# simonkosina/vbt

Measured on AMD Instinct MI355X. Metric: frames/sec end-to-end (detect+NMS+track), EfficientDet-Lite0 320x320, higher is better.
Workload: dtype int8

## Files before the change

### include/vbt_hip_diag.h

```cpp
#ifndef VBT_HIP_DIAG_H
#define VBT_HIP_DIAG_H

#include "vbt_hip.h"

#ifdef __cplusplus
extern "C" {
#endif

#define VBT_MODEL_NO_FUSION 1
#define VBT_MODEL_NO_MBCONV_FUSION 2
#define VBT_MODEL_NO_SEPCONV_FUSION 4
#define VBT_MODEL_NO_NODE_FUSION 16
#define VBT_MODEL_SINGLE_STREAM 32
#define VBT_MODEL_NO_GRAPH 64
#define VBT_MODEL_NO_HEAD_BATCHING 128
#define VBT_MODEL_NO_STEM_FUSION 256
#define VBT_MODEL_CHUNK48 2048
#define VBT_MODEL_IMAGE_BLOCKS 512
#define VBT_MODEL_TILE128 16384
#define VBT_MODEL_NO_BAND 8192
#define VBT_MODEL_NO_EXPDW 4096
#define VBT_MODEL_NO_PW_MERGE 32768
#define VBT_MODEL_NO_AUTOTUNE 8

int vbt_model_tensor_materialized(const vbt_model* m, int tensor_id);
int vbt_model_num_launches(const vbt_model* m);

int vbt_model_read_tensor(vbt_model* m, int tensor_id, int B, int8_t* host_out);

typedef struct {
  int group, alt, step;
  int chosen;
  int variant;
  int first_op, last_op;
  char family[32];
  int n_variants;
  int variants[48];
} vbt_plan_step_space;
int vbt_model_plan_space(const vbt_model* m, vbt_plan_step_space* out, int cap, int* n);

int vbt_streams_share_queue(void* a, void* b, int us, int* shared);

typedef struct {
  char name[32];
  int launches;
  double algorithmic_bytes;
  double macs;
} vbt_kernel_stat;
int vbt_model_kernel_stats(const vbt_model* m, int B, vbt_kernel_stat* out, int cap, int* n);
typedef struct {
  char family[32];
  int op, first_op, variant;
  double ms, algorithmic_bytes, macs;
} vbt_step_time;
int vbt_model_profile_steps(vbt_model* m, const uint8_t* frames_dev, int B, int reps, void* stream, vbt_step_time* out, int cap, int* n);
int vbt_model_profile_overlap(vbt_model* m, int B, int reps, int nstreams, float* single_ms, float* conc_ms, int cap, int* n);

int vbt_model_profile(vbt_model* m, const uint8_t* frames_dev, int B, int reps, void* stream,
                      double* ms_out, int cap);

int vbt_model_profile_families(vbt_model* m, int B, int reps, void* stream, double* ms_out, int cap);

int vbt_overlay_geometry(vbt_overlay* o, int32_t* out, int cap, int* n);
int vbt_overlay_hud_table(vbt_overlay* o, int32_t* out , int cap, int* P);

int vbt_mjpeg_decode_stage_ms(vbt_mjpeg_decoder* d, float* ms6);
int vbt_mjpeg_decode_entropy_info(vbt_mjpeg_decoder* d, int32_t* info4, void* stream);

#ifdef __cplusplus
}
#endif
#endif
```

### vbt_amd/_lib.py

```python
import ctypes
import os

_HERE = os.path.dirname(os.path.abspath(__file__))
LIB_PATH = os.environ.get("VBT_LIB_PATH") or os.path.join(_HERE, "libvbt_hip.so")
_lib = None

c_void_p, c_int, c_char_p, c_double = ctypes.c_void_p, ctypes.c_int, ctypes.c_char_p, ctypes.c_double


class VbtError(RuntimeError):
    pass


class VbtArgError(VbtError, ValueError):
    """VBT_ERR_ARG: the library refused an argument (also a ValueError, like the host-side checks of the wrappers)."""


class TrackerParams(ctypes.Structure):
    _fields_ = [("max_age", ctypes.c_int32), ("min_hits", ctypes.c_int32), ("delta_t", ctypes.c_int32),
                ("asso", ctypes.c_int32), ("iou_threshold", c_double), ("inertia", c_double), ("det_thresh", c_double)]


class Run(ctypes.Structure):
    _fields_ = [("clip", ctypes.c_int32), ("slot0", ctypes.c_int32), ("slot_stride", ctypes.c_int32), ("n_frames", ctypes.c_int32),
# ... 16 lines not shown
                ("strict_placement", ctypes.c_int32), ("model_flags", ctypes.c_int32), ("detection_threshold", ctypes.c_float),
                ("group", ctypes.c_int32), ("plate_diameter", c_double), ("diff_threshold", c_double), ("min_distance", c_double),
                ("tracker", TrackerParams)]


class PipelineInfo(ctypes.Structure):
    _fields_ = [(k, ctypes.c_int32) for k in ("n_slots", "n_clips", "rows_cap", "device", "depth", "ring", "defer", "tracker_inline", "image_size",
                                               "frame_count", "steps_enqueued", "placement_ok", "queue_groups_seen", "group", "next_slot")] + \
               [("reserved", ctypes.c_int32 * 1), ("det_streams", c_void_p * 8), ("copy_stream", c_void_p), ("tracker_stream", c_void_p),
                ("h2d_bytes", ctypes.c_uint64), ("step_host_ns", ctypes.c_uint64), ("step_calls", ctypes.c_uint64)]


class EvalSummary(ctypes.Structure):
    _fields_ = [(k, ctypes.c_int32) for k in ("n_rows", "n_pos", "n_neg", "n_pr", "n_roc", "flags")] + [("ap", c_double), ("auc", c_double)]


class OverlayParams(ctypes.Structure):
    _fields_ = [("trail", ctypes.c_int32), ("thickness", ctypes.c_int32), ("radius", ctypes.c_int32), ("label_scale", ctypes.c_int32),
                ("rgb", ctypes.c_uint8 * 3), ("label", ctypes.c_uint8), ("box", ctypes.c_uint8), ("reserved", ctypes.c_uint8 * 3)]


class OverlayHudParams(ctypes.Structure):
    _fields_ = [("x", ctypes.c_int32), ("y", ctypes.c_int32), ("scale", ctypes.c_int32), ("full_scale_cm", ctypes.c_int32),
                ("bg", ctypes.c_uint8 * 3), ("reserved", ctypes.c_uint8 * 5)]


class FigureParams(ctypes.Structure):
    _fields_ = [(k, ctypes.c_int32) for k in ("width", "height", "scale", "thickness", "max_figures", "max_rows", "max_phases", "reserved")]


class CurveFigureParams(ctypes.Structure):
    _fields_ = [(k, ctypes.c_int32) for k in ("width", "height", "scale", "thickness", "max_figures", "max_series", "max_points", "max_marks")]


class CurveFigureDesc(ctypes.Structure):
    _fields_ = [(k, ctypes.c_int32) for k in ("n_series", "n_marks", "legend_corner", "minor_x", "minor_y")] + \
               [("reserved", ctypes.c_int32 * 3), ("x_title", ctypes.c_char * 32), ("y_title", ctypes.c_char * 32)]


class CurveSeries(ctypes.Structure):
    _fields_ = [("n_points", ctypes.c_int32), ("colour", ctypes.c_int32), ("text", ctypes.c_char * 64)]


class CurveMark(ctypes.Structure):
    _fields_ = [("series", ctypes.c_int32), ("point", ctypes.c_int32), ("text", ctypes.c_char * 16)]


class KernelStat(ctypes.Structure):
    _fields_ = [("name", ctypes.c_char * 32), ("launches", c_int), ("algorithmic_bytes", c_double), ("macs", c_double)]


class StepTime(ctypes.Structure):
    _fields_ = [("family", ctypes.c_char * 32), ("op", c_int), ("first_op", c_int), ("variant", c_int), ("ms", c_double),
                ("algorithmic_bytes", c_double), ("macs", c_double)]


class PlanStepSpace(ctypes.Structure):
    _fields_ = [("group", c_int), ("alt", c_int), ("step", c_int), ("chosen", c_int), ("variant", c_int), ("first_op", c_int),
                ("last_op", c_int), ("family", ctypes.c_char * 32),
                ("n_variants", c_int), ("variants", c_int * 48)]


_SIGS = {
    "vbt_last_error": (c_char_p, []),
    "vbt_device_count": (c_int, []),
    "vbt_model_create": (c_int, [c_char_p, c_int, c_int, ctypes.POINTER(c_void_p)]),
    "vbt_model_create_ex": (c_int, [c_char_p, c_int, c_int, c_int, ctypes.POINTER(c_void_p)]),
    "vbt_model_destroy": (None, [c_void_p]),
    "vbt_model_tensor_materialized": (c_int, [c_void_p, c_int]),
    "vbt_model_num_launches": (c_int, [c_void_p]),
    "vbt_model_input_shape": (c_int, [c_void_p, ctypes.POINTER(c_int)]),
    "vbt_model_num_tensors": (c_int, [c_void_p]),
    "vbt_model_num_ops": (c_int, [c_void_p]),
    "vbt_model_tensor_shape": (c_int, [c_void_p, c_int, ctypes.POINTER(c_int)]),
    "vbt_detect": (c_int, [c_void_p, c_void_p, c_int, c_int, c_void_p, c_void_p, c_void_p, c_void_p, c_void_p, c_int]),
    "vbt_detect_async": (c_int, [c_void_p, c_void_p, c_int, c_void_p, c_void_p, c_void_p, c_void_p, c_void_p]),
    "vbt_detect_range_async": (c_int, [c_void_p, c_void_p, c_int, c_int, c_int, c_int, c_void_p, c_void_p, c_void_p, c_void_p, c_void_p]),
    "vbt_model_entry_steps": (c_int, [c_void_p]),
    "vbt_stream_create": (c_int, [c_int, c_void_p]),
    "vbt_stream_destroy": (c_int, [c_void_p]),
    "vbt_streams_share_queue": (c_int, [c_void_p, c_void_p, c_int, c_void_p]),
    "vbt_model_read_tensor": (c_int, [c_void_p, c_int, c_int, c_void_p]),
    "vbt_model_plan_space": (c_int, [c_void_p, c_void_p, c_int, ctypes.POINTER(c_int)]),
    "vbt_resize_frames": (c_int, [c_void_p, c_int, c_int, c_int, c_int, c_void_p, c_int, c_int, c_int, c_int, c_int, c_void_p]),
    "vbt_resize_frames_yuv": (c_int, [c_void_p, c_int, c_int, c_int, c_int, c_int, c_void_p, c_int, c_int, c_int, c_int, c_void_p]),
    "vbt_model_kernel_stats": (c_int, [c_void_p, c_int, ctypes.POINTER(KernelStat), c_int, ctypes.POINTER(c_int)]),
    "vbt_model_profile": (c_int, [c_void_p, c_void_p, c_int, c_int, c_void_p, ctypes.POINTER(c_double), c_int]),
    "vbt_model_profile_families": (c_int, [c_void_p, c_int, c_int, c_void_p, ctypes.POINTER(c_double), c_int]),
    "vbt_model_profile_steps": (c_int, [c_void_p, c_void_p, c_int, c_int, c_void_p, ctypes.POINTER(StepTime), c_int, ctypes.POINTER(c_int)]),
    "vbt_model_profile_overlap": (c_int, [c_void_p, c_int, c_int, c_int, c_void_p, c_void_p, c_int, c_void_p]),
    "vbt_tracker_create": (c_int, [c_int, c_int, ctypes.POINTER(TrackerParams), c_int, ctypes.POINTER(c_void_p)]),
    "vbt_tracker_destroy": (None, [c_void_p]),
    "vbt_tracker_reset": (c_int, [c_void_p]),
    "vbt_tracker_reset_clips": (c_int, [c_void_p, c_void_p, c_int, c_void_p]),
    "vbt_tracker_update": (c_int, [c_void_p, c_void_p, c_void_p, c_void_p, c_int]),
    "vbt_tracker_update_from_detections": (c_int, [c_void_p, c_void_p, c_void_p, c_void_p, c_void_p, ctypes.c_float, c_void_p]),
    "vbt_tracker_last_output": (c_int, [c_void_p, c_int, c_void_p, c_void_p, c_int, ctypes.POINTER(c_int)]),
    "vbt_tracker_get_trackers": (c_int, [c_void_p, c_int, c_void_p, c_void_p, c_int, ctypes.POINTER(c_int)]),
    "vbt_tracker_status": (c_int, [c_void_p, c_int] + [ctypes.POINTER(ctypes.c_int32)] * 5),
    "vbt_tracker_rows": (c_int, [c_void_p, c_int, c_void_p, c_void_p, c_int, ctypes.POINTER(c_int)]),
    "vbt_tracker_finish": (c_int, [c_void_p, c_double, c_double, c_double, c_void_p]),
    "vbt_tracker_phases": (c_int, [c_void_p, c_int, ctypes.POINTER(ctypes.c_int32), c_void_p, c_int, ctypes.POINTER(c_int)]),
    "vbt_tracker_update_from_slots": (c_int, [c_void_p, c_void_p, c_void_p, c_void_p, c_void_p, c_void_p, c_int, ctypes.c_float, c_void_p]),
    "vbt_tracker_update_from_detections_seq": (c_int, [c_void_p, c_void_p, c_void_p, c_void_p, c_int, c_void_p, c_int, ctypes.c_float, c_void_p]),
    "vbt_gather_frames": (c_int, [c_void_p, c_void_p, c_int, ctypes.c_size_t, c_void_p]),
    "vbt_tracker_summary": (c_int, [c_void_p, c_void_p, c_void_p, c_void_p, c_void_p, c_void_p, c_int]),
    "vbt_tracker_rows_all": (c_int, [c_void_p, c_void_p, c_void_p, c_int, c_void_p]),
    "vbt_tracker_live_enable": (c_int, [c_void_p, c_int, c_int, c_double, c_double, c_double]),
    "vbt_tracker_live_poll": (c_int, [c_void_p, c_int, c_void_p, c_void_p, c_int, c_void_p]),
    "vbt_tracker_live_tracks": (c_int, [c_void_p, c_int, c_int, c_void_p, c_void_p, c_void_p, c_void_p, c_void_p, c_int, c_int, ctypes.POINTER(c_int)]),
    "vbt_pipeline_default_params": (None, [ctypes.POINTER(PipelineParams)]),
    "vbt_pipeline_create": (c_int, [c_char_p, ctypes.POINTER(PipelineParams), c_void_p, ctypes.POINTER(c_void_p)]),
    "vbt_pipeline_destroy": (None, [c_void_p]),
    "vbt_pipeline_step": (c_int, [c_void_p, c_void_p, c_int, c_int, c_int, c_int, c_void_p, c_void_p, c_void_p, c_int, c_void_p]),
    "vbt_pipeline_step_runs": (c_int, [c_void_p, c_void_p, c_void_p, c_int, c_void_p, c_int, c_int, c_int, c_int, c_int, c_void_p, c_void_p, c_void_p,
                                       c_void_p, c_void_p]),
    "vbt_pipeline_set_pixel_format": (c_int, [c_void_p, c_int]),
    "vbt_pipeline_skip_frames": (c_int, [c_void_p, c_int]),
    "vbt_pipeline_set_frame_count": (c_int, [c_void_p, c_int]),
    "vbt_pipeline_reset": (c_int, [c_void_p]),
    "vbt_pipeline_join_detectors": (c_int, [c_void_p, c_void_p]),
    "vbt_pipeline_close": (c_int, [c_void_p, c_void_p, c_void_p, c_void_p, c_void_p, c_void_p, c_int]),
    "vbt_pipeline_finish": (c_int, [c_void_p]),
    "vbt_pipeline_close_clips_enable": (c_int, [c_void_p]),
    "vbt_pipeline_close_clips": (c_int, [c_void_p, c_void_p, c_int, c_void_p]),
    "vbt_pipeline_closed_clip": (c_int, [c_void_p, c_int, c_int, ctypes.POINTER(c_int), ctypes.POINTER(ClosedClip), c_void_p, c_int, c_void_p, c_int]),
    "vbt_pipeline_drain": (c_int, [c_void_p]),
    "vbt_pipeline_rows_all": (c_int, [c_void_p, c_void_p, c_void_p, c_int]),
    "vbt_pipeline_rows": (c_int, [c_void_p, c_int, c_void_p, c_void_p, c_int, ctypes.POINTER(c_int)]),
    "vbt_pipeline_detections": (c_int, [c_void_p, c_void_p, c_void_p, c_void_p, c_void_p, c_int, ctypes.POINTER(c_int)]),
    "vbt_pipeline_tracker_only_steps": (c_int, [c_void_p, c_int, c_int]),
    "vbt_pipeline_live_enable": (c_int, [c_void_p, c_int, c_int]),
    "vbt_pipeline_live_poll": (c_int, [c_void_p, c_int, c_void_p, c_void_p, c_int]),
    "vbt_pipeline_get_info": (c_int, [c_void_p, ctypes.POINTER(PipelineInfo)]),
    "vbt_pipeline_model": (c_void_p, [c_void_p, c_int]),
    "vbt_pipeline_tracker": (c_void_p, [c_void_p]),
    "vbt_track_clip": (c_int, [c_void_p, c_void_p, c_int, c_int, c_int, c_int, c_int, c_int, c_void_p, c_void_p, c_int, ctypes.POINTER(c_int)]),
    "vbt_host_alloc": (c_int, [ctypes.c_size_t, ctypes.POINTER(c_void_p)]),
    "vbt_host_free": (c_int, [c_void_p]),
    "vbt_device_alloc": (c_int, [c_int, ctypes.c_size_t, ctypes.POINTER(c_void_p)]),
    "vbt_device_free": (c_int, [c_void_p]),
    "vbt_memcpy": (c_int, [c_void_p, c_void_p, ctypes.c_size_t, c_int]),
    "vbt_stream_synchronize": (c_int, [c_void_p]),
    "vbt_device_synchronize": (c_int, [c_int]),
    "vbt_analyze": (c_int, [c_void_p, c_int, c_int, c_int, c_double, c_double, c_double, c_void_p, c_int, ctypes.POINTER(c_int), c_int]),
    "vbt_window_means": (c_int, [c_void_p, c_int, c_int, c_void_p, c_void_p, c_int]),
    "vbt_eval_create": (c_int, [c_int, c_int, c_int, ctypes.POINTER(c_void_p)]),
    "vbt_eval_destroy": (None, [c_void_p]),
    "vbt_eval_reset": (c_int, [c_void_p]),
    "vbt_eval_add_detections": (c_int, [c_void_p, c_void_p, c_void_p, c_void_p, c_int, c_void_p, c_void_p, c_void_p, c_void_p]),
    "vbt_eval_table": (c_int, [c_void_p, ctypes.POINTER(c_int), c_void_p, c_void_p, c_void_p, c_void_p, c_void_p, c_int]),
    "vbt_eval_curves": (c_int, [c_void_p, c_double, ctypes.POINTER(EvalSummary), c_void_p, c_void_p, c_void_p, c_int, c_void_p, c_void_p, c_void_p, c_int]),
    "vbt_eval_curves_from_table": (c_int, [c_void_p, c_void_p, c_int, c_double, c_int, ctypes.POINTER(EvalSummary), c_void_p, c_void_p, c_void_p, c_int,
                                           c_void_p, c_void_p, c_void_p, c_int]),
    "vbt_overlay_default_params": (None, [ctypes.POINTER(OverlayParams)]),
    "vbt_overlay_create": (c_int, [c_int, c_int, c_int, c_int, ctypes.POINTER(OverlayParams), ctypes.POINTER(c_void_p)]),
    "vbt_overlay_destroy": (None, [c_void_p]),
    "vbt_overlay_set_rows": (c_int, [c_void_p, c_void_p, c_int, c_double, c_void_p]),
    "vbt_overlay_draw": (c_int, [c_void_p, c_void_p, c_int, c_int, c_int, c_void_p]),
    "vbt_overlay_geometry": (c_int, [c_void_p, c_void_p, c_int, ctypes.POINTER(c_int)]),
    "vbt_overlay_hud_default_params": (None, [ctypes.POINTER(OverlayHudParams)]),
    "vbt_overlay_set_hud": (c_int, [c_void_p, ctypes.POINTER(OverlayHudParams), c_void_p, c_int, c_double, c_void_p]),
    "vbt_overlay_hud_table": (c_int, [c_void_p, c_void_p, c_int, ctypes.POINTER(c_int)]),
    "vbt_overlay_hud_follow": (c_int, [c_void_p, ctypes.POINTER(OverlayHudParams), c_void_p, c_int, c_double]),
    "vbt_overlay_hud_follow_update": (c_int, [c_void_p, c_int, c_void_p]),
    "vbt_overlay_hud_follow_status": (c_int, [c_void_p, ctypes.POINTER(ctypes.c_int64), ctypes.POINTER(ctypes.c_int32), ctypes.POINTER(ctypes.c_int32), c_void_p]),
# ... 74 lines not shown
```

### vbt_amd/csrc/detector.hip

```cpp
#include <algorithm>
#include <cmath>

#include "detector_model.h"
#include "op_kernels.h"

namespace vbt {

static_assert(PWM_MAX == PW_MERGE_MAX, "the planner merges as many pointwise convs as one pw_multi_kernel launch takes");


PwLaunch resolve_pw(const vbt_model* m, const Step& s, int variant, int B) {
  PwLaunch L;
  const TensorRec& to = m->tensors[m->ops[s.res_op >= 0 ? s.p_op : s.op].output];
  const long M = (long)B * to.h * to.w;
  if (s.KS64 <= 4) {
    L.form = PW_A;
    L.ms = variant >= 0 ? (variant & 1) + 1 : (M >= 32768 ? 2 : 1);
    const long waves = (M + 16 * L.ms - 1) / (16 * L.ms);
    const unsigned gx = (unsigned)((waves + 3) / 4);
    int ysplit = 1;
    while (gx * ysplit < 1024 && ysplit < s.NB) ysplit++;
    L.nb_per_y = (s.NB + ysplit - 1) / ysplit;
    L.grid = dim3(gx, (s.NB + L.nb_per_y - 1) / L.nb_per_y);
    return L;
  }
  static const int pw_force = getenv("VBT_PW_VARIANT") ? atoi(getenv("VBT_PW_VARIANT")) : -100;
  const bool f_fits = s.NB >= 2 && s.NB <= PW_F_MAX_NB;
  if (pw_force != -100 && (f_fits || (pw_force != 7 && pw_force != 8))) variant = pw_force;
  if (variant == 7 || variant == 8) {
    L.form = PW_F;
    L.ms = variant - 6;
    L.lds = s.NB * 8192;
    L.grid = dim3((unsigned)((M + 64 * L.ms - 1) / (64 * L.ms)), 1);
    if (s.NB < 2) L.refuse(VBT_ERR_ARG, "pw_conv: one output block - nothing for the all-blocks form to share");
    else if (s.NB > PW_F_MAX_NB) L.refuse(VBT_ERR_ARG, "pw_conv: %d output blocks exceed the %d whose accumulators the all-blocks form holds", s.NB, PW_F_MAX_NB);
  } else if (variant >= 3 && variant <= 6) {
    L.form = variant <= 4 ? PW_D : PW_E;
    L.ms = 2 - (variant & 1);
    L.lds = L.form == PW_E ? s.KS64 * 4096 : 0;
    L.grid = dim3((unsigned)((M + 64 * L.ms - 1) / (64 * L.ms)), (unsigned)s.NB);
    if (L.lds > 160 * 1024) L.refuse(VBT_ERR_ARG, "pw_conv: a weight panel of %d bytes does not fit the LDS", L.lds);
  } else if (variant == 2) {
    L.form = PW_C;
    L.ms = ((M + 31) / 32) * s.NB >= 512 ? 2 : 1;
    L.grid = dim3((unsigned)((M + 16 * L.ms - 1) / (16 * L.ms)), (unsigned)s.NB);
  } else {
    const unsigned gx = (unsigned)(((M + 15) / 16 + 3) / 4);
    L.nbt = std::min(s.NB, 4);
    if (gx < 512 && L.nbt > 2) L.nbt = 2;
    if (gx < 128) L.nbt = 1;
    L.grid = dim3(gx, (s.NB + L.nbt - 1) / L.nbt);
  }
  return L;
}
static int launch_pw_step(const vbt_model* m, const Step& s, int B, hipStream_t st, const int8_t* x, const int8_t* res, int8_t* out) {
  const PwLaunch L = resolve_pw(m, s, s.variant, B);
  if (L.rc) return L.report();
  const OpRec& pop = m->ops[s.res_op >= 0 ? s.p_op : s.op];
  const TensorRec& tpo = m->tensors[pop.output];
  const Epi e{s.bias, s.mult, tpo.zero_point, pop.act_min, pop.act_max, make_rq(tpo.zero_point, pop.act_min, pop.act_max)};
  const ResArgs ra{res, s.addq};
  const long M = (long)B * tpo.h * tpo.w;
  const int K = m->tensors[pop.inputs[0]].c, N = tpo.c;
#define PW(KERNEL, LDS) KERNEL<<<L.grid, 256, LDS, st>>>(x, s.wp64, e, ra, out, M, K, s.KS64, N, s.NB)
#define PW_A(KS) (L.ms == 2 ? pw_a_kernel<KS, 2><<<L.grid, 256, 0, st>>>(x, s.wp64, e, ra, out, M, K, N, s.NB, L.nb_per_y) \
                            : pw_a_kernel<KS, 1><<<L.grid, 256, 0, st>>>(x, s.wp64, e, ra, out, M, K, N, s.NB, L.nb_per_y))
  switch (L.form) {
    case PW_A: if (s.KS64 == 1) PW_A(1); else if (s.KS64 == 2) PW_A(2); else if (s.KS64 == 3) PW_A(3); else PW_A(4); break;
    case PW_D: if (L.ms == 2) PW(pw_d_kernel<2>, 0); else PW(pw_d_kernel<1>, 0); break;
    case PW_C: if (L.ms == 2) PW((pw_c_kernel<1, 2>), 0); else PW((pw_c_kernel<1, 1>), 0); break;
    case PW_E:
      if (L.ms == 2) { if (L.lds > 64 * 1024) VBT_LDS_OPT_IN(pw_e_kernel<2, 4>); PW((pw_e_kernel<2, 4>), L.lds); }
      else { if (L.lds > 64 * 1024) VBT_LDS_OPT_IN(pw_e_kernel<1, 4>); PW((pw_e_kernel<1, 4>), L.lds); }
      break;
    case PW_F:
#define PW_F_NB(NBF) (L.ms == 2 ? PW((pw_f_kernel<NBF, 2, 4>), 0) : PW((pw_f_kernel<NBF, 1, 4>), 0))
      if (s.NB == 2) PW_F_NB(2); else if (s.NB == 3) PW_F_NB(3); else if (s.NB == 4) PW_F_NB(4); else if (s.NB == 5) PW_F_NB(5); else PW_F_NB(6);
#undef PW_F_NB
      break;
    case PW_B:
      if (L.nbt == 1) PW(pw_b_kernel<1>, 0); else if (L.nbt == 2) PW(pw_b_kernel<2>, 0); else if (L.nbt == 3) PW(pw_b_kernel<3>, 0); else PW(pw_b_kernel<4>, 0);
      break;
  }
#undef PW
#undef PW_A
  return VBT_OK;
}

DwLaunch resolve_dw(const vbt_model* m, const Step& s, int variant, int B) {
  DwLaunch L;
  const OpRec& op = m->ops[s.op];
  const TensorRec& to = m->tensors[op.output];
  if (variant == 100 || variant == 101) {
    L.form = DW_TILE; L.mdw = variant == 101;
    choose_tile(to.h, to.w, op.k, op.stride, false, &L.TX, &L.TY);
    L.tiles_x = (to.w + L.TX - 1) / L.TX;
    L.tiles_y = (to.h + L.TY - 1) / L.TY;
    const int TXp = (L.TX + 3) & ~3;
    L.lds = ((TXp - 1) * op.stride + op.k) * ((L.TY - 1) * op.stride + op.k) * 80;
    L.grid = dim3((unsigned)((long)B * L.tiles_x * L.tiles_y), (unsigned)((to.c + 63) / 64));
  } else if (variant == 0) {
    L.form = DW_ROW;
    L.total = (long)B * to.h * ((to.w + 3) / 4) * (to.c / 4);
    L.grid = dim3((unsigned)((L.total + 255) / 256));
  } else {
    const long per_seg = (long)B * ((to.w + 3) / 4) * (to.c / 4);
    L.rows = std::min(variant > 0 ? variant : (int)std::min<long>(std::max<long>(to.h * per_seg / 400000, 1), 16), to.h);
    L.nseg = (to.h + L.rows - 1) / L.rows;
    L.total = per_seg * L.nseg;
    L.grid = dim3((unsigned)((L.total + 255) / 256));
  }
  return L;
}
static int launch_dw_step(const vbt_model* m, const Step& s, int B, hipStream_t st, const int8_t* x, int8_t* out, const Epi& e) {
  const DwLaunch L = resolve_dw(m, s, s.variant, B);
  if (L.rc) return L.report();
  const OpRec& op = m->ops[s.op];
  const TensorRec& ti = m->tensors[op.inputs[0]];
  const TensorRec& to = m->tensors[op.output];
  if (L.form == DW_TILE) {
    DwTileArgs a;
    a.x = x; a.out = out; a.wf = s.wf; a.bias = s.bias; a.mult = s.mult; a.wdm = s.wdm; a.bdm = s.bdm; a.mdm = s.mdm;
    a.H = ti.h; a.W = ti.w; a.C = to.c; a.OH = to.h; a.OW = to.w; a.pad_t = op.pad_t; a.pad_l = op.pad_l;
    a.TX = L.TX; a.TY = L.TY; a.tiles_x = L.tiles_x; a.tiles_y = L.tiles_y; a.zx = ti.zero_point; a.rq = e.rq;
    return launch_dw_tile(a, op.k, op.stride, L.mdw, L.grid, L.lds, st);
  }
  const unsigned pb = (unsigned)((128 + ti.zero_point) & 255);
  const unsigned pad4 = pb | (pb << 8) | (pb << 16) | (pb << 24);
#define DW_LAUNCH(KERNEL, ...)                                                                    \
  do {                                                                                            \
    if (op.k == 3 && op.stride == 1) KERNEL<3, 1><<<L.grid, 256, 0, st>>>(__VA_ARGS__);           \
    else if (op.k == 3 && op.stride == 2) KERNEL<3, 2><<<L.grid, 256, 0, st>>>(__VA_ARGS__);      \
    else if (op.k == 5 && op.stride == 1) KERNEL<5, 1><<<L.grid, 256, 0, st>>>(__VA_ARGS__);      \
    else KERNEL<5, 2><<<L.grid, 256, 0, st>>>(__VA_ARGS__);                                       \
  } while (0)
  if (L.form == DW_ROW) DW_LAUNCH(dw_kernel, x, s.wf, e, out, L.total, ti.h, ti.w, to.c, to.h, to.w, op.pad_t, op.pad_l, pad4);
  else DW_LAUNCH(dw_col_kernel, x, s.wf, e, out, L.total, ti.h, ti.w, to.c, to.h, to.w, op.pad_t, op.pad_l, pad4, L.rows, L.nseg);
#undef DW_LAUNCH
  return VBT_OK;
}

FusedPlan resolve_fused(const vbt_model* m, const Step& s, int variant, int B) {
  const FusedArgs& a = s.fa;
  const OpRec& dop = m->ops[s.d_op];
  const int k = dop.k, stride = dop.stride;
  const bool ex = s.family == F_MBCONV, ks12 = a.KSe == 1 || a.KSe == 2;
  int var = variant;
  if (var < 0) {
    var = ((m->flags & VBT_MODEL_IMAGE_BLOCKS) && !resolve_fused(m, s, 5, B).rc) ? 5 : ((m->flags & VBT_MODEL_CHUNK48) ? 9 : 1);
    const FusedPlan p17 = (m->flags & VBT_MODEL_TILE128) ? resolve_fused(m, s, 17, B) : FusedPlan{};
    if (!p17.rc && p17.L.ppw2) var |= 16;
  }
  const bool mdw = var & 1, half = var & 2;
  const bool nt3 = (var & 8) && mdw && a.nch3 > 0 && s.nbp <= 2 && a.KSe >= 1 && a.KSe <= 4;
  FusedPlan p;
  if ((var & 32) && (var & 4)) { p.refuse(VBT_ERR_ARG, "fused_mbconv: variant %d: the Toeplitz depthwise does not apply to this step", var); return p; }
  if (var & 4) {
    const int HW = a.H * a.W, OHW = a.OH * a.OW;
    if (!ex || HW > 400 || OHW > 400 || !s.ib.data) { p.refuse(VBT_ERR_ARG, "fused_mbconv: whole-image variant not applicable"); return p; }
    p.image = true;
    p.PH = std::max((a.OH - 1) * stride + k, a.pad_t + a.H);
    p.PW = std::max((a.OW - 1) * stride + k, a.pad_l + a.W);
    p.NB = (a.Cout + 63) / 64;
    const int NPGo = (OHW + 15) / 16;
    const int units = (NPGo * p.NB + IB_WAVES - 1) / IB_WAVES;
    p.maxu = units <= 2 ? 2 : units <= 3 ? 3 : 4;
    p.L.k = k; p.L.stride = stride; p.L.lds_bytes = ((HW * a.T0S + 15) & ~15) + p.PH * p.PW * FB_EST + NPGo * 16 * FB_DST + s.ib.bytes;
    if (units > 4 || p.L.lds_bytes > 160 * 1024 || s.ib.bytes > 16 * IB_NPF * IB_THREADS) p.refuse(VBT_ERR_ARG, "fused_mbconv: whole-image variant not applicable");
    return p;
  }
  p.TX = a.TX;
  p.TY = half && a.TY >= 2 ? (a.TY + 1) / 2 : a.TY;
  const bool ppw2 = (var & 16) && ex && mdw && ks12 && s.nbp <= 2 && !half;
  if (ppw2) { p.TX = 16; p.TY = 8; }
  const bool dw64 = ppw2 || (ex && mdw && a.wd64 && p.TX == 8 && p.TY == 8 && ks12 && s.nbp <= 2);
  const int est = !ex ? 0 : !nt3 ? FB_EST : dw64 ? 48 : 72;
  const bool tpz = var & 32;
  const bool tpz_ok = tpz && dw64 && a.wtz && fused_tpz_built(k, stride, s.nbp, a.KSe, ppw2) && (var & ~(1 | 8 | 16 | 32)) == 0 && nt3 == bool(var & 8) && ppw2 == bool(var & 16);
  const TpzGeom tg = tpz_ok ? tpz_geom(k, stride, ppw2 ? 2 : 1, nt3 ? 3 : 4) : TpzGeom{};
  const int e_bytes = tpz_ok ? tg.e_bytes + 8 * tg.DSK : -1;
  p.tiles_x = (a.OW + p.TX - 1) / p.TX;
  p.tiles_y = (a.OH + p.TY - 1) / p.TY;
  p.L = FusedLaunch{k, stride, s.nbp, ex, mdw, nt3, ppw2, dw64, fused_tile_lds(a, k, stride, p.TX, p.TY, est, ppw2 ? 2 : 1, s.nbp, e_bytes),
                    (unsigned)((long)B * p.tiles_x * p.tiles_y), tpz_ok};
  if (ppw2 && (a.OW < 16 || a.OH < 8 || !a.wd64)) p.refuse(VBT_ERR_ARG, "fused_mbconv: the 128-pixel variant needs maps of at least 16 x 8");
  else if (ppw2 && p.L.lds_bytes > 64 * 1024) p.refuse(VBT_ERR_ARG, "fused_mbconv: 128-pixel tile needs %d bytes of LDS", p.L.lds_bytes);
  else if (tpz && !tpz_ok) p.refuse(VBT_ERR_ARG, "fused_mbconv: variant %d: the Toeplitz depthwise does not apply to this step", var);
  else if (tpz && p.L.lds_bytes > 64 * 1024) p.refuse(VBT_ERR_ARG, "fused_mbconv: the Toeplitz depthwise tile needs %d bytes of LDS", p.L.lds_bytes);
  return p;
}
static int launch_fused_step(const vbt_model* m, const Step& s, FusedArgs a, int B, hipStream_t st) {
  const FusedPlan p = resolve_fused(m, s, s.variant, B);
  if (p.rc) return p.report();
  if (p.image) return launch_mbconv_image(a, s.ib, p.L.k, p.L.stride, p.maxu, p.PW, p.PH, p.NB, p.L.lds_bytes, B, st);
  a.TX = p.TX; a.TY = p.TY; a.tiles_x = p.tiles_x; a.tiles_y = p.tiles_y;
  return launch_fused_block(a, p.L, st);
}

ExpDwLaunch resolve_expdw(const vbt_model*, const Step& s, int variant, int B) {
  static const int xd_force = getenv("VBT_XD_VARIANT") ? atoi(getenv("VBT_XD_VARIANT")) : -100;
  if (xd_force != -100 && (xd_force < 100 || (s.xd2_ok && (xd_force < 200 ? s.xd2_gpw > 0 : s.xd2_gpw16 > 0)))) variant = std::min(xd_force, xd_force / 100 * 100 + s.xd.nchunks);
  ExpDwLaunch L;
  if (s.xd2_ok && (variant >= 100 || variant < 0)) {
    if (variant >= 200 && s.xd2_gpw16 == 0) { L.refuse(VBT_ERR_ARG, "expand + depthwise: plan asks for the 16-wave form on a step that does not support it"); return L; }
    if (variant >= 100 && variant < 200 && s.xd2_gpw == 0) { L.refuse(VBT_ERR_ARG, "expand + depthwise: plan asks for the 8-wave form on a step that does not support it"); return L; }
    const ExpDw2Args& a = s.xd2;
    L.second = true;
    L.nw = (variant >= 200 || (variant < 0 && s.xd2_gpw16 > 0)) ? 16 : 8;
    L.gpw = L.nw == 16 ? s.xd2_gpw16 : s.xd2_gpw;
    L.cpw = std::min(variant >= 100 ? variant % 100 : std::max(1, (a.nchunks * a.nbands * B + 1023) / 1024), a.nchunks);
    L.grid = (unsigned)(B * ((a.nchunks + L.cpw - 1) / L.cpw) * a.nbands);
    L.lds = s.xd2_lds;
    return L;
  }
  if (variant >= 100) { L.refuse(VBT_ERR_ARG, "expand + depthwise: plan asks for the second kernel form on a step that does not support it"); return L; }
  const ExpDwArgs& a = s.xd;
  L.cpw = variant > 0 ? variant : std::max(1, (a.nchunks * a.nbands * B + 511) / 512);
  L.grid = (unsigned)(B * ((a.nchunks + L.cpw - 1) / L.cpw) * a.nbands);
  L.lds = s.lds_bytes;
  return L;
}
static int launch_expdw_step(const vbt_model* m, const Step& s, int B, hipStream_t st, const int8_t* x, int8_t* out) {
  const ExpDwLaunch L = resolve_expdw(m, s, s.variant, B);
  if (L.rc) return L.report();
  const OpRec& dop = m->ops[s.d_op];
  if (L.second) {
    ExpDw2Args a = s.xd2;
    a.x = x; a.out = out; a.cpw = L.cpw;
    return launch_expdw2(a, dop.k, dop.stride, (a.Cin + 63) / 64, L.nw, L.gpw, L.grid, L.lds, st);
  }
  ExpDwArgs a = s.xd;
  a.x = x; a.out = out; a.cpw = L.cpw;
  return launch_expdw(a, dop.k, dop.stride, (a.Cin + 63) / 64, L.grid, L.lds, st);
}

static bool band_chainable(const Step& s) {
  if (s.members.empty()) return s.bd_args.wpc != nullptr;
  for (const Step& ms : s.members)
    if (!ms.bd_args.wpc) return false;
  return true;
}
BandLaunch resolve_band(const vbt_model* m, const Step& s, int variant, int) {
  BandLaunch L;
  const bool can = band_chainable(s);
  if (variant < -1 || variant > 1) { L.refuse(VBT_ERR_ARG, "fused_sepconv_band: no kernel form %d", variant); return L; }
  if (variant == 1 && !can) { L.refuse(VBT_ERR_ARG, "fused_sepconv_band: plan asks for the chained form on a step that does not support it"); return L; }
  static const int bd_force = getenv("VBT_BAND_VARIANT") ? atoi(getenv("VBT_BAND_VARIANT")) : -100;
  if (bd_force == 0 || (bd_force == 1 && can)) variant = bd_force;
  L.chained = variant == 1 || (variant < 0 && can && m->max_batch > 8);
  if (s.members.empty()) L.lds = band_lds(s.bd_args, L.chained);
  for (const Step& ms : s.members) L.lds = std::max(L.lds, band_lds(ms.bd_args, L.chained));
  if (L.lds > 160 * 1024) L.refuse(VBT_ERR_ARG, "fused_sepconv_band: a band of %d bytes does not fit the LDS", L.lds);
  return L;
}

StemLaunch resolve_stemblk(const vbt_model*, const Step&, int variant, int) {
  StemLaunch L;
  if (variant < -1 || variant > 1) { L.refuse(VBT_ERR_ARG, "fused_stem_block: no kernel form %d", variant); return L; }
  L.direct = variant == 1;
  return L;
}

int launch_step(vbt_model* m, const Step& s, int B, hipStream_t st, const uint8_t* frames, float* boxes, float* scores, float* classes,
                int* counts, int boff) {
  if (m->pool_dirty) { const int rc = flush_uploads(m); if (rc) return rc; }
  const OpRec& op = m->ops[s.op];
  const TensorRec& to = m->tensors[op.output];
// ... 356 lines not shown
```

### vbt_amd/csrc/detector_model.h

```cpp
#pragma once
#include <cstdarg>
#include <map>
#include <tuple>
#include <vector>

#include "dev_mem.h"
#include "hip_handles.h"
#include "launchers.h"
#include "plan_geom.h"

namespace vbt {

enum Family { F_STEM = 0, F_PW, F_DW, F_ADD, F_MAXPOOL, F_RESIZE, F_POST, F_MBCONV, F_SEPCONV, F_NODE, F_MULTI, F_STEMBLK, F_EXPDW, F_BAND, F_COUNT };
inline const char* const kFamilyName[F_COUNT] = {"stem_conv_mfma_i8", "pw_conv_mfma_i8", "dw_conv_f32acc", "add_requant",
                                                 "maxpool3x3s2", "resize_nn", "decode_nms", "fused_mbconv", "fused_sepconv", "fused_bifpn_node", "fused_heads_multi",
                                                 "fused_stem_block", "fused_expand_dw", "fused_sepconv_band"};

constexpr int PW_MERGE_MAX = 8;

struct Cost {
  double alg_bytes_per_frame = 0, weight_bytes = 0, macs_per_frame = 0;
  Cost& operator+=(const Cost& o) { alg_bytes_per_frame += o.alg_bytes_per_frame; weight_bytes += o.weight_bytes; macs_per_frame += o.macs_per_frame; return *this; }
};

struct Step {
  int op;
  int family;
  long* wp = nullptr;
  v4i* wp64 = nullptr;
  int KS64 = 0;
  int res_op = -1;
  long* wdm = nullptr;
  int* bdm = nullptr;
  float* mdm = nullptr;
  float* wf = nullptr;
  int* bias = nullptr;
  float* mult = nullptr;
  int KS = 0, NB = 0;
  AddQ addq = {0, 0, 0, 0, 0, 0, 0};
  Cost cost;
  int e_op = -1, d_op = -1, p_op = -1, a_op = -1;
  int sum_op = -1;
  int src_tensor[3] = {-1, -1, -1};
  FusedArgs fa;
  int nbp = 0, lds_bytes = 0;
  int variant = -1;
  double tuned_ms = 0;
  std::vector<Step> members;
  FusedArgs* d_multi = nullptr;
  StemBlockArgs sb;
  BandArgs bd_args;
  BandArgs* d_band = nullptr;
  int band_tiles = 0;
  ExpDwArgs xd;
  ExpDw2Args xd2;
  bool xd2_ok = false;
  int xd2_lds = 0, xd2_gpw = 0, xd2_gpw16 = 0;
  ImageBundle ib = {nullptr, 0, 0, 0, 0, 0, 0, 0};
};

struct Alt {
  std::vector<Step> steps;
  std::vector<int> hidden;
  double ms = 0;
};
struct Group {
  std::vector<Alt> alts;
  int chosen = 0;
};

}

struct vbt_model {
  vbt_model() = default;
  ~vbt_model() {
    for (int k = 0; k < 4; k++) { sub_streams[k].reset(); ev_join[k].reset(); }
    ev_fork.reset();
    clear_graphs();
    cap_stream.reset();
  }
  vbt::Header hdr;
  std::vector<vbt::TensorRec> tensors;
  std::vector<vbt::OpRec> ops;
  std::vector<uint8_t> blob;
  int device = 0, max_batch = 0;
  std::vector<int8_t*> tptr;
  std::vector<size_t> telems;
  int8_t* arena = nullptr;
  uint8_t* frames_stage = nullptr;
  vbt::DevBuf<unsigned char> out_block;
  float* out_boxes = nullptr;
  float* out_scores = nullptr;
  float* out_classes = nullptr;
  int* out_counts = nullptr;
  vbt::PinnedBuf<unsigned char> out_host;
  size_t out_bytes = 0;
  float* d_anchors = nullptr;
  unsigned char* d_luts = nullptr;
  std::vector<float> post_tables_host;
  std::vector<vbt::Step> steps;
  std::vector<vbt::Group> groups;
  std::vector<vbt::Step> op_steps;
  std::vector<char> materialized;
  int flags = 0;
  int n_sub = 1;
  vbt::Stream sub_streams[4];
  vbt::Event ev_fork, ev_join[4];
  struct GraphKey {
    const void* frames; void* boxes; void* scores; void* classes; void* counts; int B;
    bool operator<(const GraphKey& o) const {
      return std::tie(frames, boxes, scores, classes, counts, B) < std::tie(o.frames, o.boxes, o.scores, o.classes, o.counts, o.B);
    }
  };
  std::map<GraphKey, hipGraphExec_t> graphs;
  void clear_graphs() {
    for (auto& kv : graphs) (void)hipGraphExecDestroy(kv.second);
    graphs.clear();
  }
  vbt::Stream cap_stream;
  int graph_max_batch = 0;
  bool ran_eager = false;
  std::vector<vbt::DevBuf<char>> owned;
  struct PoolChunk { vbt::DevBuf<char> dev; std::vector<char> host; size_t used, flushed; };
  std::vector<PoolChunk> pool;
  bool pool_dirty = false;
  int last_B = 0;
};

namespace vbt {

int upload_bytes(vbt_model* m, const void* src, size_t bytes, void** dev);
template <typename T>
int upload(vbt_model* m, const std::vector<T>& h, T** d) { return upload_bytes(m, h.data(), h.size() * sizeof(T), (void**)d); }
int flush_uploads(vbt_model* m);

int build_plan(vbt_model* m);
void finalize_plan(vbt_model* m);

struct Verdict {
  int rc = VBT_OK; char why[160] = "";
  void refuse(int code, const char* fmt, ...) { va_list ap; va_start(ap, fmt); vsnprintf(why, sizeof(why), fmt, ap); va_end(ap); rc = code; }
  int report() const { set_error("%s", why); return rc; }
};
enum PwForm { PW_A, PW_B, PW_C, PW_D, PW_E, PW_F };
constexpr int PW_F_MAX_NB = 6;
struct PwLaunch : Verdict { PwForm form = PW_B; int ms = 1, nbt = 1, nb_per_y = 0, lds = 0; dim3 grid; };
enum DwForm { DW_ROW, DW_COL, DW_TILE };
struct DwLaunch : Verdict {
  DwForm form = DW_COL; bool mdw = false; int TX = 0, TY = 0, tiles_x = 0, tiles_y = 0, lds = 0, rows = 0, nseg = 0; long total = 0; dim3 grid;
};
struct FusedPlan : Verdict {
  bool image = false; int PW = 0, PH = 0, NB = 0, maxu = 0;
  int TX = 0, TY = 0, tiles_x = 0, tiles_y = 0; FusedLaunch L{};
};
struct ExpDwLaunch : Verdict {
  bool second = false; int cpw = 1, nw = 0, gpw = 0, lds = 0; unsigned grid = 0;
};
struct BandLaunch : Verdict { bool chained = false; int lds = 0; };
struct StemLaunch : Verdict { bool direct = false; };
PwLaunch resolve_pw(const vbt_model* m, const Step& s, int variant, int B);
DwLaunch resolve_dw(const vbt_model* m, const Step& s, int variant, int B);
FusedPlan resolve_fused(const vbt_model* m, const Step& s, int variant, int B);
ExpDwLaunch resolve_expdw(const vbt_model* m, const Step& s, int variant, int B);
BandLaunch resolve_band(const vbt_model* m, const Step& s, int variant, int B);
StemLaunch resolve_stemblk(const vbt_model* m, const Step& s, int variant, int B);

int launch_step(vbt_model* m, const Step& s, int B, hipStream_t st, const uint8_t* frames, float* boxes, float* scores, float* classes,
                int* counts, int boff = 0);
inline int launch_step_staged(vbt_model* m, const Step& s, int B, hipStream_t st) {
  return launch_step(m, s, B, st, m->frames_stage, m->out_boxes, m->out_scores, m->out_classes, m->out_counts);
}
int enqueue_forward(vbt_model* m, const uint8_t* frames_dev, int B, hipStream_t st, float* boxes, float* scores, float* classes, int* counts,
                    const Event* evs);

}
```

### vbt_amd/csrc/detector_plan.hip

```cpp
#include <algorithm>
#include <chrono>
#include <cmath>
#include <functional>
#include <string>

#include "detector_model.h"

namespace vbt {

static bool fence_on() {
  static int v = -1;
  if (v < 0) { const char* e = getenv("VBT_DEBUG_FENCE"); v = (e && e[0] == '1') ? 1 : 0; }
  return v == 1;
}
static hipError_t fenced_malloc(vbt_model* m, void** out, size_t bytes) {
  const size_t G = 2u << 20;
  const size_t total = fence_on() ? (bytes + G - 1) / G * G : bytes;
  DevBuf<char> base;
  const hipError_t e = base.alloc(total);
  if (e != hipSuccess) return e;
  *out = base.get() + ((total - bytes) & ~(size_t)255);
  m->owned.push_back(std::move(base));
  return hipSuccess;
}
// ... 17 lines not shown
  return VBT_OK;
}
int flush_uploads(vbt_model* m) {
  if (!m->pool_dirty) return VBT_OK;
  for (auto& c : m->pool)
    if (c.used > c.flushed) {
      VBT_HIP_CHECK(hipMemcpy(c.dev.get() + c.flushed, c.host.data() + c.flushed, c.used - c.flushed, hipMemcpyHostToDevice));
      c.flushed = c.used;
    }
  m->pool_dirty = false;
  return VBT_OK;
}

int upload_bytes(vbt_model* m, const void* src, size_t n, void** d) {
  size_t bytes = std::max<size_t>(n, 16);
  if (fence_on()) {
    VBT_HIP_CHECK(fenced_malloc(m, d, bytes + 64));
    if (n) VBT_HIP_CHECK(hipMemcpy(*d, src, n, hipMemcpyHostToDevice));
    return VBT_OK;
  }
  char* host = nullptr;
  int rc = pool_alloc(m, bytes + 64, d, &host);
  if (rc) return rc;
  if (n) memcpy(host, src, n);
  return VBT_OK;
}

static double time_step(vbt_model* m, const Step& s, int B, int reps) {
  static int nconc = -1;
  static hipStream_t cs[4] = {nullptr, nullptr, nullptr, nullptr};
  if (nconc < 0) {
    const char* e = getenv("VBT_AUTOTUNE_CONCURRENCY");
    nconc = e ? std::max(1, std::min(4, atoi(e))) : 1;
    if (nconc > 1)
      for (int i = 0; i < nconc; i++) (void)hipStreamCreateWithFlags(&cs[i], hipStreamNonBlocking);
  }
  Event e0, e1;
  if (e0.create(hipEventDefault) != hipSuccess || e1.create(hipEventDefault) != hipSuccess) return 1e30;
  float ms = 1e30f;
  int rc = VBT_OK;
  if (nconc <= 1) {
    rc = launch_step_staged(m, s, B, nullptr);
    (void)hipEventRecord(e0.get(), nullptr);
    for (int r = 0; r < reps && !rc; r++)
      rc = launch_step_staged(m, s, B, nullptr);
    (void)hipEventRecord(e1.get(), nullptr);
    if (hipEventSynchronize(e1.get()) != hipSuccess || hipEventElapsedTime(&ms, e0.get(), e1.get()) != hipSuccess) ms = 1e30f;
    ms /= reps;
  } else {
    (void)hipDeviceSynchronize();
    for (int i = 0; i < nconc && !rc; i++)
      rc = launch_step_staged(m, s, B, cs[i]);
    (void)hipDeviceSynchronize();
    auto t0 = std::chrono::steady_clock::now();
    for (int r = 0; r < reps; r++)
      for (int i = 0; i < nconc && !rc; i++)
        rc = launch_step_staged(m, s, B, cs[i]);
    (void)hipDeviceSynchronize();
    ms = (float)(std::chrono::duration<double, std::milli>(std::chrono::steady_clock::now() - t0).count() / (reps * nconc));
  }
  return rc ? 1e30 : ms;
}

static bool is_fused_tile(int family) { return family == F_MBCONV || family == F_SEPCONV || family == F_NODE; }
static bool variant_ok(const vbt_model* m, const Step& st, int v) {
  if (st.family == F_PW) return !st.members.empty() || !resolve_pw(m, st, v, m->max_batch).rc;
  if (is_fused_tile(st.family)) return !resolve_fused(m, st, v, m->max_batch).rc;
  if (st.family == F_BAND) return !resolve_band(m, st, v, m->max_batch).rc;
  if (st.family == F_STEMBLK) return !resolve_stemblk(m, st, v, m->max_batch).rc;
  return st.family != F_EXPDW || !resolve_expdw(m, st, v, m->max_batch).rc;
}

static std::vector<int> candidate_variants(const vbt_model* m, const Step& st) {
  std::vector<int> cand{-1};
  const OpRec& op = m->ops[st.op];
  if (st.family == F_DW) {
    cand = {0};
    for (int r : {1, 2, 4, 8, 16})
      if (r <= m->tensors[op.output].h) cand.push_back(r);
    if (m->tensors[op.output].c % 8 == 0) { cand.push_back(100); cand.push_back(101); }
  } else if (st.family == F_PW && st.KS64 <= 4) {
    cand = {0, 1};
  } else if (st.family == F_PW) {
    cand = {-1, 2, 3, 4, 5, 6, 7, 8};
  } else if (is_fused_tile(st.family)) {
    cand = {0, 1, 3, 5};
    if (st.family == F_MBCONV && st.fa.nch3 > 0 && st.nbp <= 2 && st.fa.KSe >= 1 && st.fa.KSe <= 4) { cand.push_back(9); cand.push_back(11); }
    if (st.family == F_MBCONV && st.nbp <= 2 && (st.fa.KSe == 1 || st.fa.KSe == 2)) {
      cand.push_back(17);
      if (st.fa.nch3 > 0) cand.push_back(25);
    }
    if (st.family == F_MBCONV && st.fa.wtz) cand.insert(cand.end(), {33, 41, 49, 57});
  } else if (st.family == F_MULTI) {
    cand = {0, 1};
  } else if (st.family == F_EXPDW) {
    cand.clear();
    for (int cpw : {1, 2, 3, 4, 6})
      if (cpw <= st.xd.nchunks) cand.push_back(cpw);
    if (st.xd2_ok)
      for (int cpw : {1, 2, 3, 4, 6})
        if (cpw <= st.xd.nchunks) {
          if (st.xd2_gpw > 0) cand.push_back(100 + cpw);
          if (st.xd2_gpw16 > 0) cand.push_back(200 + cpw);
        }
  } else if (st.family == F_BAND) {
    cand = {-1, 0, 1};
  } else if (st.family == F_STEMBLK) {
    cand = {-1, 0, 1};
  }
  cand.erase(std::remove_if(cand.begin(), cand.end(), [&](int v) { return !variant_ok(m, st, v); }), cand.end());
  return cand;
}

static void autotune(vbt_model* m) {
  const int B = (m->max_batch + m->n_sub - 1) / m->n_sub, reps = 4;
  for (Group& g : m->groups) {
    bool single = g.alts.size() == 1 && g.alts[0].steps.size() == 1;
    if (single) {
      int f = g.alts[0].steps[0].family;
      if (f != F_DW && f != F_PW) continue;
    }
    for (Alt& a : g.alts) {
      a.ms = 0;
      for (Step& st : a.steps) {
        const std::vector<int> cand = candidate_variants(m, st);
        double best = 1e30;
        int bestv = -1;
        for (int v : cand) {
          Step t = st;
          t.variant = v;
          double ms = time_step(m, t, B, reps);
          if (getenv("VBT_AUTOTUNE_VERBOSE") && cand.size() > 1 && atoi(getenv("VBT_AUTOTUNE_VERBOSE")) > 1)
            fprintf(stderr, "[autotune]   op %d %s v%d %.1fus\n", st.op, kFamilyName[st.family], v, ms * 1e3);
          if (ms < best) { best = ms; bestv = v; }
        }
        st.variant = bestv;
        st.tuned_ms = best;
        a.ms += best;
      }
    }
    int bi = 0;
    for (size_t i = 1; i < g.alts.size(); i++)
      if (g.alts[i].ms < g.alts[bi].ms) bi = (int)i;
    g.chosen = bi;
    if (getenv("VBT_AUTOTUNE_VERBOSE")) {
      const Step& f = g.alts[0].steps[0];
      const TensorRec& to = m->tensors[m->ops[g.alts[0].steps.back().op].output];
      fprintf(stderr, "[autotune] op %3d.. out %3dx%3dx%4d :", f.op, to.h, to.w, to.c);
      for (size_t i = 0; i < g.alts.size(); i++) {
        fprintf(stderr, " alt%zu%s %.1fus(", i, (int)i == bi ? "*" : "", g.alts[i].ms * 1e3);
        for (const Step& st : g.alts[i].steps) fprintf(stderr, "%s:v%d=%.1f ", kFamilyName[st.family], st.variant, st.tuned_ms * 1e3);
        fprintf(stderr, ")");
      }
      fprintf(stderr, "\n");
    }
  }
  (void)hipDeviceSynchronize();
}

static PlanShape plan_shape(const vbt_model* m) {
  PlanShape shape;
  for (const Group& g : m->groups) {
    std::vector<std::vector<PlanStepShape>> alts;
    for (const Alt& a : g.alts) {
      std::vector<PlanStepShape> steps;
      for (const Step& st : a.steps) {
        PlanStepShape ps;
// ... 13 lines not shown
  return shape;
}
static bool load_plan(vbt_model* m, const char* path) {
  const PlanShape shape = plan_shape(m);
  std::vector<PlanChoice> sel;
  std::string note;
  if (!parse_plan_file(path, shape, &sel, &note)) {
    if (note != "no such file") fprintf(stderr, "[vbt] plan %s: %s - plan refused, re-tuning\n", path, note.c_str());
    return false;
  }
  for (size_t gi = 0; gi < m->groups.size(); gi++) {
    m->groups[gi].chosen = sel[gi].chosen;
    Alt& a = m->groups[gi].alts[(size_t)sel[gi].chosen];
    for (size_t i = 0; i < a.steps.size(); i++) a.steps[i].variant = sel[gi].variants[i];
  }
  return true;
}
static void save_plan(const vbt_model* m, const char* path) {
  FILE* f = fopen(path, "w");
  if (!f) return;
  fprintf(f, "VBTPLAN2 %d\n", (int)m->groups.size());
  for (const Group& g : m->groups) {
    const Alt& a = g.alts[g.chosen];
    fprintf(f, "%d %d", g.chosen, (int)a.steps.size());
    for (const Step& st : a.steps) fprintf(f, " %s:%d", kFamilyName[st.family], st.variant);
    fprintf(f, "\n");
  }
  fclose(f);
}

}

using namespace vbt;

extern "C" {

int vbt_model_create(const char* path, int device, int max_batch, vbt_model** out) {
  const char* nf = getenv("VBT_FUSION_FLAGS");
  return vbt_model_create_ex(path, device, max_batch, nf ? atoi(nf) : VBT_MODEL_DEFAULT_FLAGS, out);
}

int vbt_model_tensor_materialized(const vbt_model* m, int id) {
  if (!m || id < 0 || id >= (int)m->tensors.size()) { set_error("bad tensor id"); return VBT_ERR_ARG; }
  return m->materialized[id] ? 1 : 0;
}

int vbt_model_num_launches(const vbt_model* m) { return m ? (int)m->steps.size() : VBT_ERR_ARG; }

int vbt_model_plan_space(const vbt_model* m, vbt_plan_step_space* out, int cap, int* n) {
  if (!m || !n || cap < 0 || (cap > 0 && !out)) { set_error("vbt_model_plan_space: bad argument"); return VBT_ERR_ARG; }
  const PlanShape shape = plan_shape(m);
  int total = 0;
  for (const auto& alts : shape.groups)
    for (const auto& steps : alts) total += (int)steps.size();
  *n = total;
  if (total > cap) { set_error("plan space: %d steps, buffer holds %d", total, cap); return VBT_ERR_CAPACITY; }
  int i = 0;
  for (size_t gi = 0; gi < shape.groups.size(); gi++)
    for (size_t ai = 0; ai < shape.groups[gi].size(); ai++)
      for (size_t si = 0; si < shape.groups[gi][ai].size(); si++, i++) {
        const PlanStepShape& ps = shape.groups[gi][ai][si];
        vbt_plan_step_space& o = out[i];
        memset(&o, 0, sizeof(o));
        if (ps.variants.size() > sizeof(o.variants) / sizeof(o.variants[0])) {
          set_error("plan space: group %zu alternative %zu step %zu has %zu variants", gi, ai, si, ps.variants.size());
          return VBT_ERR_CAPACITY;
        }
        o.group = (int)gi; o.alt = (int)ai; o.step = (int)si;
        o.chosen = m->groups[gi].chosen == (int)ai;
        const Step& st = m->groups[gi].alts[ai].steps[si];
        o.variant = st.variant;
        o.first_op = (int)m->ops.size(); o.last_op = -1;
        std::function<void(const Step&)> span = [&](const Step& s) {
          for (int op : {s.op, s.e_op, s.d_op, s.p_op, s.a_op, s.sum_op})
            if (op >= 0) { o.first_op = std::min(o.first_op, op); o.last_op = std::max(o.last_op, op); }
          for (const Step& mb : s.members) span(mb);
        };
        span(st);
        snprintf(o.family, sizeof(o.family), "%s", ps.family.c_str());
        o.n_variants = (int)ps.variants.size();
        std::copy(ps.variants.begin(), ps.variants.end(), o.variants);
      }
  return VBT_OK;
}

int vbt_model_create_ex(const char* path, int device, int max_batch, int flags, vbt_model** out) {
  if (!path || !out || max_batch < 1) { set_error("vbt_model_create: bad argument"); return VBT_ERR_ARG; }
  *out = nullptr;
  vbt_model* m = new vbt_model();
  {
    ContainerData cd;
    std::string why;
    if (!read_container(path, &cd, &why)) { delete m; set_error("%s", why.c_str()); return VBT_ERR_IO; }
    m->hdr = cd.hdr;
    m->tensors.swap(cd.tensors);
    m->ops.swap(cd.ops);
    m->blob.swap(cd.blob);
  }
  m->device = device;
  m->max_batch = max_batch;
  m->flags = flags;
  if (int drc = use_device("vbt_model_create", device, false)) { delete m; return drc; }
  int rc = VBT_OK;
  auto fail = [&](int code) { vbt_model_destroy(m); return code; };
  if (hipSetDevice(device) != hipSuccess) { set_error("hipSetDevice(%d) failed", device); return fail(VBT_ERR_HIP); }
  size_t total = 0;
  m->telems.resize(m->tensors.size());
  std::vector<size_t> off(m->tensors.size());
  for (size_t i = 0; i < m->tensors.size(); i++) {
    const TensorRec& t = m->tensors[i];
    m->telems[i] = (size_t)t.h * t.w * t.c;
    off[i] = total;
    size_t bytes = (int)i == m->hdr.input_tensor ? 0 : m->telems[i] * max_batch;
    total += (bytes + 255) / 256 * 256 + 256;
  }
  if (fenced_malloc(m, (void**)&m->arena, total + 4096) != hipSuccess) { set_error("hipMalloc(%zu) for activations failed", total); return fail(VBT_ERR_HIP); }
  (void)hipMemset(m->arena, 0, total + 4096);
  m->tptr.resize(m->tensors.size());
  for (size_t i = 0; i < m->tensors.size(); i++) m->tptr[i] = m->arena + off[i];
  size_t fbytes = (size_t)max_batch * m->hdr.image_size * m->hdr.image_size * 3;
  const int md = m->hdr.max_detections;
  m->out_bytes = (size_t)max_batch * (md * 24 + 4);
  if (fenced_malloc(m, (void**)&m->frames_stage, fbytes + 64) != hipSuccess || m->out_block.alloc(m->out_bytes) != hipSuccess ||
      m->out_host.alloc(m->out_bytes) != hipSuccess) {
    set_error("hipMalloc for staging buffers failed");
    return fail(VBT_ERR_HIP);
  }
  m->out_boxes = (float*)m->out_block.get();
  m->out_scores = m->out_boxes + (size_t)max_batch * md * 4;
  m->out_classes = m->out_scores + (size_t)max_batch * md;
  m->out_counts = (int*)(m->out_classes + (size_t)max_batch * md);
  if ((rc = build_plan(m)) != VBT_OK) return fail(rc);
  for (const OpRec& op : m->ops)
    if (op.type == OP_POSTPROCESS) {
      std::vector<float> an((const float*)(m->blob.data() + op.aux_off), (const float*)(m->blob.data() + op.aux_off) + (size_t)m->hdr.num_anchors * 4);
      if ((size_t)op.aux2_off + VBT_POST_TABLE_BYTES > m->blob.size()) { set_error("post-process tables truncated"); return fail(VBT_ERR_IO); }
      std::vector<unsigned char> lut(m->blob.data() + op.aux2_off, m->blob.data() + op.aux2_off + VBT_POST_TABLE_BYTES);
      const float* sv = (const float*)(lut.data() + 6144);
      if (sv[0] != sv[1] || sv[2] != sv[3]) { set_error("post-process: y_scale != x_scale or h_scale != w_scale"); return fail(VBT_ERR_ARG); }
      {
        const int nl = op.n_inputs / 2;
        const TensorRec& tc = m->tensors[op.inputs[0]];
        const TensorRec& tb = m->tensors[op.inputs[nl]];
        for (int l = 1; l < nl; l++) {
          const TensorRec &c2 = m->tensors[op.inputs[l]], &b2 = m->tensors[op.inputs[nl + l]];
          if (c2.scale != tc.scale || c2.zero_point != tc.zero_point || b2.scale != tb.scale || b2.zero_point != tb.zero_point) {
            set_error("post-process: head outputs of level %d are quantised differently from level 0", l);
            return fail(VBT_ERR_ARG);
          }
        }
        const float* st_score = (const float*)lut.data();
        const float* st_box = st_score + 256;
        const double* st_dq = (const double*)(lut.data() + 2048);
        const double* st_ex = st_dq + 256;
        for (int q = -128; q < 128; q++) {
          const float x = tc.scale * (float)(q - tc.zero_point);
          float y = 256.0f / (1.0f + expf(-x));
          y = y < 0.0f ? 0.0f : (y > 255.0f ? 255.0f : y);
          const float want_score = (1.0f / 256.0f) * (float)lrintf(y);
          const float want_box = tb.scale * (float)(q - tb.zero_point);
          const double want_dq = (double)want_box / (double)sv[0];
          const double want_ex = exp((double)want_box / (double)sv[2]);
          if (st_score[q + 128] != want_score || st_box[q + 128] != want_box || st_dq[q + 128] != want_dq || st_ex[q + 128] != want_ex) {
            set_error("post-process: stored table entry %d differs from the one derived from the tensor scales", q);
            return fail(VBT_ERR_ARG);
          }
// ... 73 lines not shown
```

### vbt_amd/csrc/fused_block.h

```cpp
#pragma once
#include "tpz_geom.h"

struct FusedArgs {
  const int8_t* x;
  int8_t* out;
  int H, W, Cin, OH, OW, Cout;
  int pad_t, pad_l;
  int TX, TY, tiles_x, tiles_y;
  int T0S;
  int nchunks;
  int zx;
  const long* we;
  const int* be;
  const float* me;
  int KSe, ze, loe, hie;
  Rq rqe;
  const long* we3;
  const long* wdm3;
  const v4i* wp3;
  int nch3, KSp3;
  const float* wd;
  const int* bd;
  const float* md;
  int zd, lod, hid;
  Rq rqd;
  const long* wdm;
  const int* bdm;
  const v4i* wd64;
  const long* wd64c;
  const unsigned* wtz;
  const v4i* wp;
  const int* bp;
  const float* mp;
  int KSp, zo, lop, hip;
  Rq rqp;
  int has_res;
  AddQ resq;
  int n_src;
  const int8_t* src[3];
  int sh[3], sw[3], smode[3], spt[3], spl[3];
  int chain;
  AddQ sumq, preq;
};

__device__ __forceinline__ unsigned node_sum4(const unsigned u[3], const FusedArgs& a) {
  if (a.chain == 0) return addq4(u[0], u[1], a.sumq);
  const unsigned p = addq4(u[0], u[1], a.preq);
  return a.chain == 1 ? addq4(p, u[2], a.sumq) : addq4(u[2], p, a.sumq);
}

typedef unsigned short v2u16 __attribute__((ext_vector_type(2)));
__device__ __forceinline__ unsigned pk_max_u16(unsigned a, unsigned b) {
  v2u16 x, y;
  __builtin_memcpy(&x, &a, 4);
  __builtin_memcpy(&y, &b, 4);
  v2u16 r = __builtin_elementwise_max(x, y);
  unsigned o;
  __builtin_memcpy(&o, &r, 4);
  return o;
}

constexpr int FB_EST = 80;
constexpr int FB_DST = 80;

template <int KK, int S, int NBP, bool EXPAND, bool MDW, int KSE = 0, int NT = 4, int PPW = 1, bool DW64 = false, bool TPZ = false>
__device__ __forceinline__ void fused_block_body(const FusedArgs& a, int tile, unsigned char* fb_smem) {
  static_assert(PPW == 1 || MDW, "128-pixel tiles exist for the matrix-pipe depthwise only");
  static_assert(!DW64 || (EXPAND && MDW && (KK == 3 || KK == 5)), "DW64: fused expand blocks, 3x3 / 5x5");
  static_assert(!TPZ || (DW64 && (S == 1 || S == 2) && (NT == 3 || NT == 4) && NBP <= 2 && (KSE == 1 || KSE == 2)), "TPZ: a form of DW64");
  constexpr TpzGeom TG = TPZ ? tpz_geom(KK, S, PPW, NT) : TpzGeom{};
  constexpr int KT2 = (S * (S - 1) + KK + 1) / 2;
  const int tid = threadIdx.x, wave = tid >> 6, lane = tid & 63, r = lane & 15, g = lane >> 4;
  const int trow = fdiv_small(tile, frcp(a.tiles_x));
  const int tx = tile - trow * a.tiles_x;
  const int bimg = fdiv_small(trow, frcp(a.tiles_y));
  const int ty = trow - bimg * a.tiles_y;
  const long b = bimg;
  const int oy0 = ty * a.TY, ox0 = tx * a.TX;
  const int TXp = (a.TX + 3) & ~3;
  const int HWx = (TXp - 1) * S + KK, HWy = (a.TY - 1) * S + KK, NPh = HWx * HWy;
  const int iy0 = oy0 * S - a.pad_t, ix0 = ox0 * S - a.pad_l;
  const float rcp_hwx = frcp(HWx), rcp_txp = frcp(TXp);
  unsigned char* T0 = fb_smem;
  unsigned char* E = T0 + ((NPh * a.T0S + 15) & ~15);
  constexpr int EST = (EXPAND && NT == 3) ? (DW64 ? 48 : 72) : FB_EST;
  unsigned char* D = E + (EXPAND ? (TPZ ? TG.e_bytes : ((NPh * EST + 15) & ~15)) : 0);
  bool stage_p = false;
  if constexpr (!EXPAND && NBP <= 2) stage_p = a.nchunks == 1;
  unsigned char* WPS = D + 64 * PPW * FB_DST;
  unsigned char* BPS = WPS + NBP * 4096;

  bool summed = false;
  if constexpr (!EXPAND) summed = a.n_src > 0;
  if (summed) {
    const int nd = a.Cin >> 2;
    const unsigned zb4 = (unsigned)(a.zx & 255) * 0x01010101u;
    const int pstep = fdiv_small(256, frcp(nd));
    int p = fdiv_small(tid, frcp(nd));
    const int cd = tid - p * nd;
    const bool up2[3] = {a.H == 2 * a.sh[0] && a.W == 2 * a.sw[0], a.H == 2 * a.sh[1] && a.W == 2 * a.sw[1], a.H == 2 * a.sh[2] && a.W == 2 * a.sw[2]};
    for (; tid < pstep * nd && p < NPh; p += pstep) {
      const int hy = fdiv_small(p, rcp_hwx), hx = p - hy * HWx;
      const int iy = iy0 + hy, ix = ix0 + hx;
      unsigned v = zb4;
      if (iy >= 0 && iy < a.H && ix >= 0 && ix < a.W) {
        unsigned us[3] = {0u, 0u, 0u};
#pragma unroll
        for (int j = 0; j < 3; j++) {
          if (j < a.n_src) {
            const int8_t* sb = a.src[j] + b * (long)a.sh[j] * a.sw[j] * a.Cin + 4 * cd;
            unsigned u;
            if (a.smode[j] == 0) {
              u = *(const unsigned*)(sb + ((long)iy * a.sw[j] + ix) * a.Cin);
            } else if (a.smode[j] == 1) {
              int yy, xx;
              if (up2[j]) { yy = iy >> 1; xx = ix >> 1; }
              else { yy = (iy * a.sh[j]) / a.H; xx = (ix * a.sw[j]) / a.W; }
              u = *(const unsigned*)(sb + ((long)yy * a.sw[j] + xx) * a.Cin);
            } else {
              unsigned tv[9];
#pragma unroll
              for (int ky = 0; ky < 3; ky++) {
                const int yy = iy * 2 + ky - a.spt[j];
                const int yc = min(max(yy, 0), a.sh[j] - 1);
#pragma unroll
                for (int kx = 0; kx < 3; kx++) {
                  const int xx = ix * 2 + kx - a.spl[j];
                  const int xc = min(max(xx, 0), a.sw[j] - 1);
                  const unsigned t = *(const unsigned*)(sb + ((long)yc * a.sw[j] + xc) * a.Cin);
                  tv[ky * 3 + kx] = (yy == yc && xx == xc) ? (t ^ 0x80808080u) : 0u;
                }
              }
              unsigned lo = 0u, hi = 0u;
#pragma unroll
              for (int q = 0; q < 9; q++) {
                const unsigned l = tv[q] & 0x00FF00FFu, h = (tv[q] >> 8) & 0x00FF00FFu;
                lo = pk_max_u16(lo, l);
                hi = pk_max_u16(hi, h);
              }
              u = (lo | (hi << 8)) ^ 0x80808080u;
            }
            us[j] = u;
          }
        }
        v = node_sum4(us, a);
      }
      *(unsigned*)(T0 + p * a.T0S + 4 * cd) = v;
    }
  } else {
    if (!EXPAND && (a.Cin & 15) == 0) {
// ... 260 lines not shown
      if (PREF_DW || (!EXPAND && c == 0)) {
#pragma unroll
        for (int mi = 0; mi < KT; mi++) wreg[mi] = wpre[mi];
        bqm = bpre;
        mum = mpre;
      } else if (cg_active) {
#pragma unroll
        for (int mi = 0; mi < KT; mi++) wreg[mi] = wm[mi * 64];
        bqm = *(const int4*)(a.bdm + c * CH + 16 * wave + 4 * g);
        mum = *(const float4*)(a.md + c * CH + 16 * wave + 4 * g);
      }
      const unsigned char* lane_base = Ein + 16 * wave + 8 * (g & 1);
      const int hi_half = g >> 1;
#pragma unroll
      for (int pg = 0; pg < 4 * PPW; pg += 2) {
        if (!cg_active) break;
        v4i dqa = v4i_from(bqm), dqb = v4i_from(bqm);
        const unsigned char* pba = lane_base + hbase[pg] * est;
        const unsigned char* pbb = lane_base + hbase[pg + 1] * est;
#pragma unroll
        for (int mi = 0; mi < KT; mi++) {
          const int ta = 2 * mi, tb = (2 * mi + 1 < KK * KK) ? 2 * mi + 1 : 2 * mi;
          const int offa = ((ta / KK) * HWx + (ta % KK)) * est, offb = ((tb / KK) * HWx + (tb % KK)) * est;
          const int off = hi_half ? offb : offa;
          long bva = *(const long*)(pba + off);
          long bvb = *(const long*)(pbb + off);
          dqa = __builtin_amdgcn_mfma_i32_16x16x32_i8(wreg[mi], bva, dqa, 0, 0, 0);
          dqb = __builtin_amdgcn_mfma_i32_16x16x32_i8(wreg[mi], bvb, dqb, 0, 0, 0);
        }
        *(unsigned*)(D + (pg * 16 + r) * FB_DST + 16 * wave + 4 * g) = rq_pack_b(dqa, mum, a.rqd);
        *(unsigned*)(D + ((pg + 1) * 16 + r) * FB_DST + 16 * wave + 4 * g) = rq_pack_b(dqb, mum, a.rqd);
      }
    } else if (dw_active) {
      const unsigned char* Ein = EXPAND ? E + 4 * cq : T0 + 64 * c + 4 * cq;
      const int est = EXPAND ? EST : a.T0S;
      constexpr int IW = 3 * S + KK;
      const int Cp = a.nchunks * 64;
      const float* wd = a.wd + c * 64 + 4 * cq;
      float dacc[4][4];
#pragma unroll
      for (int o = 0; o < 4; o++)
#pragma unroll
        for (int j = 0; j < 4; j++) dacc[o][j] = 0.0f;
#pragma unroll
      for (int ky = 0; ky < KK; ky++) {
        float4 wr[KK];
#pragma unroll
        for (int kx = 0; kx < KK; kx++) wr[kx] = *(const float4*)(wd + (long)(ky * KK + kx) * Cp);
        const unsigned char* rowp = Ein + ((sy * S + ky) * HWx + sx * S) * est;
#pragma unroll
        for (int j = 0; j < IW; j++) {
          unsigned u = *(const unsigned*)(rowp + j * est) ^ 0x80808080u;
          float f0 = (float)(u & 255u), f1 = (float)((u >> 8) & 255u), f2 = (float)((u >> 16) & 255u), f3 = (float)(u >> 24);
#pragma unroll
          for (int kx = 0; kx < KK; kx++) {
            if ((j - kx) >= 0 && (j - kx) % S == 0 && (j - kx) / S < 4) {
              const int o = (j - kx) / S;
              dacc[o][0] = __builtin_fmaf(f0, wr[kx].x, dacc[o][0]);
              dacc[o][1] = __builtin_fmaf(f1, wr[kx].y, dacc[o][1]);
              dacc[o][2] = __builtin_fmaf(f2, wr[kx].z, dacc[o][2]);
              dacc[o][3] = __builtin_fmaf(f3, wr[kx].w, dacc[o][3]);
            }
          }
        }
      }
      const int4 bq = *(const int4*)(a.bd + c * 64 + 4 * cq);
      const float4 mu = *(const float4*)(a.md + c * 64 + 4 * cq);
#pragma unroll
      for (int o = 0; o < 4; o++) {
        v4i ai = {(int)dacc[o][0], (int)dacc[o][1], (int)dacc[o][2], (int)dacc[o][3]};
        unsigned dd = rq_pack_i(ai, bq, mu, a.rqd);
        *(unsigned*)(D + (sy * TXp + sx + o) * FB_DST + 4 * cq) = dd;
      }
    }
    __syncthreads();
    {
      v4i bv[PPW];
#pragma unroll
      for (int pp = 0; pp < PPW; pp++) {
        const int slot = (wave * PPW + pp) * 16 + r;
        bv[pp] = *(const v4i*)(D + (TPZ ? tpz_d_slot(TG, PPW, FB_DST, slot) : slot * FB_DST) + 16 * g);
      }
#pragma unroll
      for (int nb = 0; nb < NBP; nb++) {
        const v4i* w = stage_p ? (const v4i*)WPS + (nb * 4) * 64 + lane
                               : (NT == 3 ? a.wp3 + ((long)(nb * a.KSp3 + c) * 4) * 64 : a.wp + ((long)(nb * a.KSp + c) * 4) * 64) + lane;
#pragma unroll
        for (int t = 0; t < 4; t++) {
          const v4i wv = w[t * 64];
#pragma unroll
          for (int pp = 0; pp < PPW; pp++) acc[pp][nb][t] = __builtin_amdgcn_mfma_i32_16x16x64_i8(wv, bv[pp], acc[pp][nb][t], 0, 0, 0);
        }
      }
    }
    if (!EXPAND && c + 1 < nch) __syncthreads();
  }

#pragma unroll
  for (int pp = 0; pp < PPW; pp++) {
  const int slot = (wave * PPW + pp) * 16 + r;
  const int py = fdiv_small(slot, rcp_txp), px = slot - py * TXp;
  const int oy = oy0 + py, ox = ox0 + px;
  if (py < a.TY && px < a.TX && oy < a.OH && ox < a.OW) {
    const unsigned char* skip = T0 + ((py + a.pad_t) * HWx + (px + a.pad_l)) * a.T0S;
    int8_t* orow = a.out + ((b * a.OH + oy) * (long)a.OW + ox) * a.Cout;
#pragma unroll
    for (int nb = 0; nb < NBP; nb++) {
      const int c0 = nb * 64 + 16 * g;
      if (c0 >= a.Cout) continue;
      unsigned d[4];
#pragma unroll
      for (int t = 0; t < 4; t++) {
        int4 bb;
        float4 mu;
        if (stage_p) {
          bb = *(const int4*)(BPS + 4 * (c0 + 4 * t));
          mu = *(const float4*)(BPS + NBP * 256 + 4 * (c0 + 4 * t));
        } else {
          bb = *(const int4*)(a.bp + c0 + 4 * t);
          mu = *(const float4*)(a.mp + c0 + 4 * t);
        }
        unsigned dq = rq_pack_i(acc[pp][nb][t], bb, mu, a.rqp);
        if (a.has_res) {
          const unsigned xs = *(const unsigned*)(skip + min(c0 + 4 * t, a.Cin - 4));
          dq = addq4(dq, xs, a.resq);
        }
        d[t] = dq;
      }
      int8_t* o = orow + c0;
      if ((a.Cout & 15) == 0) {
        *(uint4*)o = make_uint4(d[0], d[1], d[2], d[3]);
      } else if ((a.Cout & 3) == 0) {
#pragma unroll
        for (int t = 0; t < 4; t++)
          if (c0 + 4 * t < a.Cout) *(unsigned*)(o + 4 * t) = d[t];
      } else {
#pragma unroll
        for (int t = 0; t < 4; t++)
#pragma unroll
          for (int j = 0; j < 4; j++)
            if (c0 + 4 * t + j < a.Cout) o[4 * t + j] = (int8_t)(d[t] >> (8 * j));
      }
    }
  }
  }
}


#ifndef FB_MINW
#define FB_MINW 1
#endif
template <int KK, int S, int NBP, bool EXPAND, bool MDW, int KSE = 0, int NT = 4, int PPW = 1, bool DW64 = false, bool TPZ = false>
__global__ __launch_bounds__(256, FB_MINW) void fused_block_kernel(FusedArgs a) {
  extern __shared__ __attribute__((aligned(16))) unsigned char fb_smem_dyn[];
  fused_block_body<KK, S, NBP, EXPAND, MDW, KSE, NT, PPW, DW64, TPZ>(a, blockIdx.x, fb_smem_dyn);
}

struct MultiTiles {
  int n;
  int start[13];
};
template <int KK, int S, int NBP, bool EXPAND, bool MDW>
__global__ __launch_bounds__(256, FB_MINW) void fused_block_multi_kernel(const FusedArgs* __restrict__ args, MultiTiles mt) {
  extern __shared__ __attribute__((aligned(16))) unsigned char fb_smem_dyn[];
  int p = 0;
#pragma unroll
  for (int i = 1; i < 12; i++)
    if (i < mt.n && (int)blockIdx.x >= mt.start[i]) p = i;
  fused_block_body<KK, S, NBP, EXPAND, MDW>(args[p], (int)blockIdx.x - mt.start[p], fb_smem_dyn);
}

struct DwTileArgs {
  const int8_t* x;
  int8_t* out;
  const float* wf;
  const int* bias;
  const float* mult;
  const long* wdm;
  const int* bdm;
  const float* mdm;
  int H, W, C, OH, OW, pad_t, pad_l, TX, TY, tiles_x, tiles_y, zx;
  Rq rq;
};

template <int KK, int S, bool MDW>
__global__ __launch_bounds__(256) void dw_tile_kernel(DwTileArgs a) {
  extern __shared__ __attribute__((aligned(16))) unsigned char dt_smem[];
  constexpr int TS = 80;
  const int tid = threadIdx.x;
  int tile = blockIdx.x;
  const int tx = tile % a.tiles_x;
  tile /= a.tiles_x;
  const int ty = tile % a.tiles_y;
  const long b = tile / a.tiles_y;
  const int c0 = blockIdx.y * 64;
  const int cvalid = min(64, a.C - c0);
  const int oy0 = ty * a.TY, ox0 = tx * a.TX;
  const int TXp = (a.TX + 3) & ~3;
  const int HWx = (TXp - 1) * S + KK, HWy = (a.TY - 1) * S + KK, NPh = HWx * HWy;
  const int iy0 = oy0 * S - a.pad_t, ix0 = ox0 * S - a.pad_l;
  {
    const int ng = (cvalid + 7) >> 3;
    const unsigned long long zb = (unsigned long long)(a.zx & 255) * 0x0101010101010101ull;
    const int8_t* xb = a.x + b * (long)a.H * a.W * a.C + c0;
    const int pstep = 256 / ng;
    int p = tid / ng;
    const int sg = tid - p * ng;
    int hy = p / HWx, hx = p - hy * HWx;
    for (; tid < pstep * ng && p < NPh; p += pstep) {
      const int iy = iy0 + hy, ix = ix0 + hx;
      unsigned long long v = zb;
      if (iy >= 0 && iy < a.H && ix >= 0 && ix < a.W) v = *(const unsigned long long*)(xb + ((long)iy * a.W + ix) * a.C + 8 * sg);
      *(unsigned long long*)(dt_smem + p * TS + 8 * sg) = v;
      hx += pstep;
      while (hx >= HWx) { hx -= HWx; hy++; }
    }
  }
  if constexpr (MDW) {
    constexpr int KT = (KK * KK + 1) / 2;
    const int wave = tid >> 6, lane = tid & 63, r = lane & 15, g = lane >> 4;
    const long* wm = a.wdm + ((long)(blockIdx.y * 4 + wave) * KT) * 64 + lane;
    long wreg[KT];
#pragma unroll
    for (int mi = 0; mi < KT; mi++) wreg[mi] = wm[mi * 64];
    const int cbase = c0 + 16 * wave + 4 * g;
    const int4 bqm = *(const int4*)(a.bdm + cbase);
    const float4 mum = *(const float4*)(a.mdm + cbase);
    const float rcp_txp = 1.0f / (float)TXp;
    __syncthreads();
    if (16 * wave >= cvalid) return;
    const unsigned char* lane_base = dt_smem + 16 * wave + 8 * (g & 1);
    const int hi_half = g >> 1;
#pragma unroll
    for (int pg = 0; pg < 4; pg++) {
      const int slot = pg * 16 + r;
      const int sq = fdiv_small(slot, rcp_txp);
      const int py = min(sq, a.TY - 1), px = slot - sq * TXp;
      const unsigned char* pb = lane_base + ((py * S) * HWx + px * S) * TS;
// ... 70 lines not shown
```

### vbt_amd/csrc/k_fused_mbconv.hip

```cpp
#include "launchers.h"

namespace vbt {

#define FB_P2(KK, S, NBP, KSE)                                                                                      \
  do {                                                                                                              \
    if (L.nt3) fused_block_kernel<KK, S, NBP, true, true, KSE, 3, 2, true><<<grid, 256, L.lds_bytes, st>>>(a);      \
    else fused_block_kernel<KK, S, NBP, true, true, KSE, 4, 2, true><<<grid, 256, L.lds_bytes, st>>>(a);            \
  } while (0)
#define FB_P2K(KK, S)                                                                                               \
  do {                                                                                                              \
    if (L.nbp == 1 && a.KSe == 1) FB_P2(KK, S, 1, 1);                                                               \
    else if (L.nbp == 1) FB_P2(KK, S, 1, 2);                                                                        \
    else if (a.KSe == 1) FB_P2(KK, S, 2, 1);                                                                        \
    else FB_P2(KK, S, 2, 2);                                                                                        \
  } while (0)
#define FB_DW64(KK, S, NBP)                                                                                                                    \
  do {                                                                                                                                         \
    if (L.nt3 && a.KSe == 1) fused_block_kernel<KK, S, (NBP <= 2 ? NBP : 1), true, true, 1, 3, 1, true><<<grid, 256, L.lds_bytes, st>>>(a);    \
    else if (L.nt3) fused_block_kernel<KK, S, (NBP <= 2 ? NBP : 1), true, true, 2, 3, 1, true><<<grid, 256, L.lds_bytes, st>>>(a);            \
    else if (a.KSe == 1) fused_block_kernel<KK, S, (NBP <= 2 ? NBP : 1), true, true, 1, 4, 1, true><<<grid, 256, L.lds_bytes, st>>>(a);       \
    else fused_block_kernel<KK, S, (NBP <= 2 ? NBP : 1), true, true, 2, 4, 1, true><<<grid, 256, L.lds_bytes, st>>>(a);                       \
  } while (0)
#define FB_LAUNCH(KK, S, NBP)                                                                                                                          \
  do {                                                                                                                                                 \
    if (L.dw64) FB_DW64(KK, S, NBP);                                                                                                                   \
    else if (L.mdw && L.nt3 && NBP <= 2 && a.KSe == 1) fused_block_kernel<KK, S, (NBP <= 2 ? NBP : 1), true, true, 1, 3><<<grid, 256, L.lds_bytes, st>>>(a); \
    else if (L.mdw && L.nt3 && NBP <= 2 && a.KSe == 2) fused_block_kernel<KK, S, (NBP <= 2 ? NBP : 1), true, true, 2, 3><<<grid, 256, L.lds_bytes, st>>>(a); \
    else if (L.mdw && L.nt3 && NBP <= 2 && a.KSe == 3) fused_block_kernel<KK, S, (NBP <= 2 ? NBP : 1), true, true, 3, 3><<<grid, 256, L.lds_bytes, st>>>(a); \
    else if (L.mdw && L.nt3 && NBP <= 2 && a.KSe == 4) fused_block_kernel<KK, S, (NBP <= 2 ? NBP : 1), true, true, 4, 3><<<grid, 256, L.lds_bytes, st>>>(a); \
    else if (L.mdw && a.KSe == 1) fused_block_kernel<KK, S, NBP, true, true, 1><<<grid, 256, L.lds_bytes, st>>>(a);                                   \
    else if (L.mdw && a.KSe == 2) fused_block_kernel<KK, S, NBP, true, true, 2><<<grid, 256, L.lds_bytes, st>>>(a);                                   \
    else if (L.mdw && a.KSe == 3) fused_block_kernel<KK, S, NBP, true, true, 3><<<grid, 256, L.lds_bytes, st>>>(a);                                   \
    else if (L.mdw && a.KSe == 4) fused_block_kernel<KK, S, NBP, true, true, 4><<<grid, 256, L.lds_bytes, st>>>(a);                                   \
    else if (L.mdw) fused_block_kernel<KK, S, NBP, true, true><<<grid, 256, L.lds_bytes, st>>>(a);                                                    \
    else fused_block_kernel<KK, S, NBP, true, false><<<grid, 256, L.lds_bytes, st>>>(a);                                                              \
  } while (0)
#define FB_NBP(KK, S)                                      \
  do {                                                     \
    switch (L.nbp) {                                       \
      case 1: FB_LAUNCH(KK, S, 1); break;                  \
      case 2: FB_LAUNCH(KK, S, 2); break;                  \
      case 3: FB_LAUNCH(KK, S, 3); break;                  \
      default: FB_LAUNCH(KK, S, 5); break;                 \
    }                                                      \
  } while (0)

int launch_fused_mbconv_tpz(const FusedArgs& a, const FusedLaunch& L, hipStream_t st);

int launch_fused_mbconv(const FusedArgs& a, const FusedLaunch& L, hipStream_t st) {
  if (L.tpz) return launch_fused_mbconv_tpz(a, L, st);
  const dim3 grid(L.grid);
  if (L.ppw2) {
    if (L.k == 3 && L.stride == 1) FB_P2K(3, 1);
    else if (L.k == 3 && L.stride == 2) FB_P2K(3, 2);
    else if (L.k == 5 && L.stride == 1) FB_P2K(5, 1);
    else FB_P2K(5, 2);
    return VBT_OK;
  }
  if (L.k == 3 && L.stride == 1) FB_NBP(3, 1);
  else if (L.k == 3 && L.stride == 2) FB_NBP(3, 2);
  else if (L.k == 5 && L.stride == 1) FB_NBP(5, 1);
  else FB_NBP(5, 2);
  return VBT_OK;
}

}
```

### vbt_amd/csrc/launchers.h

```cpp
#pragma once
#include "dev_common.h"

namespace vbt {
#include "fused_block.h"
#include "stem_block.h"
#include "image_block.h"
#include "expdw_block.h"
#include "expdw2_block.h"
#include "band_block.h"

struct FusedLaunch {
  int k, stride, nbp;
  bool expand;
  bool mdw;
  bool nt3;
  bool ppw2;
  bool dw64;
  int lds_bytes;
  unsigned grid;
  bool tpz = false;
};
static inline bool fused_tpz_built(int k, int stride, int nbp, int kse, bool ppw2) {
  return (k == 3 && stride == 2 && nbp == 1 && kse == 1) || (k == 3 && stride == 1 && nbp == 1 && kse == 1) ||
         (k == 5 && stride == 2 && nbp == 1 && kse == 1 && !ppw2) || (k == 5 && stride == 1 && nbp == 1 && kse == 2);
}
int launch_fused_block(const FusedArgs& a, const FusedLaunch& L, hipStream_t st);
int launch_fused_multi(const FusedArgs* d_args, const MultiTiles& mt, int k, int stride, int nbp, bool mdw, int lds_bytes, unsigned grid,
                       hipStream_t st);
int launch_dw_tile(const DwTileArgs& a, int k, int stride, bool mdw, dim3 grid, int lds_bytes, hipStream_t st);
int launch_mbconv_image(const FusedArgs& a, const ImageBundle& wb, int k, int stride, int maxu, int PW, int PH, int NB, int lds_bytes, int B,
                        hipStream_t st);
int launch_band_one(const BandArgs& a, bool chained, unsigned grid, int lds_bytes, hipStream_t st);
int launch_band_multi(const BandArgs* d_probs, const MultiTiles& mt, int C, bool chained, unsigned grid, int lds_bytes, hipStream_t st);
int launch_expdw(const ExpDwArgs& a, int k, int stride, int KS64, unsigned grid, int lds_bytes, hipStream_t st);
int launch_expdw2(const ExpDw2Args& a, int k, int stride, int KS64, int nw, int gpw, unsigned grid, int lds_bytes, hipStream_t st);
int launch_stem_block(const StemBlockArgs& a, bool direct, unsigned grid, hipStream_t st);

}
```

### vbt_amd/csrc/op_kernels.h

```cpp
#pragma once
#include "launchers.h"

namespace vbt {

struct ResArgs {
  const int8_t* res;
  AddQ q;
};
__device__ __forceinline__ void store_tile_r(const v4i acc[4], const Epi& e, const ResArgs& ra, int8_t* __restrict__ out, long m, int N,
                                             int nb, int g) {
  int c0 = nb * 64 + 16 * g;
  if (c0 >= N) return;
  unsigned d[4];
#pragma unroll
  for (int t = 0; t < 4; t++) {
    int4 b = *(const int4*)(e.bias + c0 + 4 * t);
    float4 mu = *(const float4*)(e.mult + c0 + 4 * t);
    d[t] = rq_pack_i(acc[t], b, mu, e.rq);
  }
  if (ra.res) {
    const int8_t* r = ra.res + m * N + c0;
#pragma unroll
    for (int t = 0; t < 4; t++)
      if (c0 + 4 * t < N) d[t] = addq4(d[t], *(const unsigned*)(r + 4 * t), ra.q);
  }
  int8_t* o = out + m * N + c0;
  if ((N & 15) == 0) {
    *(uint4*)o = make_uint4(d[0], d[1], d[2], d[3]);
  } else if ((N & 3) == 0) {
#pragma unroll
    for (int t = 0; t < 4; t++)
      if (c0 + 4 * t < N) *(unsigned*)(o + 4 * t) = d[t];
  } else {
#pragma unroll
    for (int t = 0; t < 4; t++)
#pragma unroll
      for (int j = 0; j < 4; j++)
        if (c0 + 4 * t + j < N) o[4 * t + j] = (int8_t)(d[t] >> (8 * j));
  }
}
struct EpiRegs {
  int4 b[4];
  float4 mu[4];
  unsigned res[4];
};
__device__ __forceinline__ void load_epi(EpiRegs& er, const Epi& e, const ResArgs& ra, long m, int N, int nb, int g) {
  const int c0 = min(nb * 64 + 16 * g, ((N + 15) & ~15) - 16);
#pragma unroll
  for (int t = 0; t < 4; t++) {
    er.b[t] = *(const int4*)(e.bias + c0 + 4 * t);
    er.mu[t] = *(const float4*)(e.mult + c0 + 4 * t);
    er.res[t] = 0u;
  }
  if (ra.res) {
    const int8_t* r = ra.res + m * N + nb * 64 + 16 * g;
#pragma unroll
    for (int t = 0; t < 4; t++)
      if (nb * 64 + 16 * g + 4 * t < N) er.res[t] = *(const unsigned*)(r + 4 * t);
  }
}
__device__ __forceinline__ void store_tile_e(const v4i acc[4], const EpiRegs& er, const Epi& e, const ResArgs& ra, int8_t* __restrict__ out,
                                             long m, int N, int nb, int g) {
  int c0 = nb * 64 + 16 * g;
  if (c0 >= N) return;
  unsigned d[4];
#pragma unroll
  for (int t = 0; t < 4; t++) {
    d[t] = rq_pack_i(acc[t], er.b[t], er.mu[t], e.rq);
    if (ra.res) d[t] = addq4(d[t], er.res[t], ra.q);
  }
  int8_t* o = out + m * N + c0;
  if ((N & 15) == 0) {
    *(uint4*)o = make_uint4(d[0], d[1], d[2], d[3]);
  } else if ((N & 3) == 0) {
#pragma unroll
    for (int t = 0; t < 4; t++)
      if (c0 + 4 * t < N) *(unsigned*)(o + 4 * t) = d[t];
  } else {
#pragma unroll
    for (int t = 0; t < 4; t++)
#pragma unroll
      for (int j = 0; j < 4; j++)
        if (c0 + 4 * t + j < N) o[4 * t + j] = (int8_t)(d[t] >> (8 * j));
  }
}
__device__ __forceinline__ v4i ld16(const int8_t* p) {
  v4i v;
  __builtin_memcpy(&v, p, 16);
  return v;
}

template <int KS, int MS>
__global__ __launch_bounds__(256) void pw_a_kernel(const int8_t* __restrict__ x, const v4i* __restrict__ wp, Epi e, ResArgs ra,
                                                   int8_t* __restrict__ out, long M, int K, int N, int NB,
                                                   int nb_per_y) {
  const int wave = threadIdx.x >> 6, lane = threadIdx.x & 63;
  const int r = lane & 15, g = lane >> 4;
  const long m0 = ((long)blockIdx.x * 4 + wave) * (16 * MS);
  if (m0 >= M) return;
  v4i a[MS][KS];
#pragma unroll
  for (int ms = 0; ms < MS; ms++) {
    long m = min(m0 + 16 * ms + r, M - 1);
    const int8_t* p = x + m * K + 16 * g;
#pragma unroll
    for (int ks = 0; ks < KS; ks++) a[ms][ks] = ld16(p + 64 * ks);
  }
  const int nb0 = blockIdx.y * nb_per_y, nb1 = min(nb0 + nb_per_y, NB);
  for (int nb = nb0; nb < nb1; nb++) {
    v4i acc[MS][4];
#pragma unroll
    for (int ms = 0; ms < MS; ms++)
#pragma unroll
      for (int t = 0; t < 4; t++) acc[ms][t] = (v4i){0, 0, 0, 0};
    const v4i* w = wp + (long)nb * KS * 4 * 64 + lane;
#pragma unroll
    for (int ks = 0; ks < KS; ks++)
#pragma unroll
      for (int t = 0; t < 4; t++) {
        v4i wv = w[(ks * 4 + t) * 64];
#pragma unroll
        for (int ms = 0; ms < MS; ms++)
          acc[ms][t] = __builtin_amdgcn_mfma_i32_16x16x64_i8(wv, a[ms][ks], acc[ms][t], 0, 0, 0);
      }
#pragma unroll
    for (int ms = 0; ms < MS; ms++) {
      long m = m0 + 16 * ms + r;
      if (m < M) store_tile_r(acc[ms], e, ra, out, m, N, nb, g);
    }
  }
}

template <int NBT>
__global__ __launch_bounds__(256) void pw_b_kernel(const int8_t* __restrict__ x, const v4i* __restrict__ wp, Epi e, ResArgs ra,
                                                   int8_t* __restrict__ out, long M, int K, int KS, int N, int NB) {
  const int wave = threadIdx.x >> 6, lane = threadIdx.x & 63;
  const int r = lane & 15, g = lane >> 4;
  const long m0 = ((long)blockIdx.x * 4 + wave) * 16;
  if (m0 >= M) return;
  const int nb0 = blockIdx.y * NBT;
  v4i acc[NBT][4];
#pragma unroll
  for (int i = 0; i < NBT; i++)
#pragma unroll
    for (int t = 0; t < 4; t++) acc[i][t] = (v4i){0, 0, 0, 0};
  const int8_t* p = x + min(m0 + r, M - 1) * K + 16 * g;
  EpiRegs er[NBT];
#pragma unroll
  for (int i = 0; i < NBT; i++) load_epi(er[i], e, ra, min(m0 + r, M - 1), N, min(nb0 + i, NB - 1), g);
#pragma unroll 4
  for (int ks = 0; ks < KS; ks++) {
    v4i av = ld16(p + 64 * ks);
#pragma unroll
    for (int i = 0; i < NBT; i++) {
      int nb = min(nb0 + i, NB - 1);
      const v4i* w = wp + ((long)(nb * KS + ks) * 4) * 64 + lane;
#pragma unroll
      for (int t = 0; t < 4; t++) acc[i][t] = __builtin_amdgcn_mfma_i32_16x16x64_i8(w[t * 64], av, acc[i][t], 0, 0, 0);
    }
  }
  long m = m0 + r;
  if (m < M) {
#pragma unroll
    for (int i = 0; i < NBT; i++)
      if (nb0 + i < NB) store_tile_e(acc[i], er[i], e, ra, out, m, N, nb0 + i, g);
  }
// ... 118 lines not shown
#pragma unroll
    for (int t = 0; t < 4; t++) {
      const v4i wv = wbuf[ks & 1][t][lane];
#pragma unroll
      for (int s = 0; s < MS; s++) acc[s][t] = __builtin_amdgcn_mfma_i32_16x16x64_i8(wv, a_cur[s], acc[s][t], 0, 0, 0);
    }
    wbuf[(ks + 1) & 1][wave][lane] = wreg;
#pragma unroll
    for (int s = 0; s < MS; s++) a_cur[s] = a_nxt[s];
    __syncthreads();
  }
#pragma unroll
  for (int s = 0; s < MS; s++) {
    const long m = m0 + 16 * s + r;
    if (m < M) store_tile_e(acc[s], er[s], e, ra, out, m, N, nb, g);
  }
}

template <int MS, int PD>
__global__ __launch_bounds__(256) void pw_e_kernel(const int8_t* __restrict__ x, const v4i* __restrict__ wp, Epi e, ResArgs ra,
                                                   int8_t* __restrict__ out, long M, int K, int KS, int N, int NB) {
  extern __shared__ __attribute__((aligned(16))) unsigned char pwe_smem[];
  v4i* wpanel = (v4i*)pwe_smem;
  const int tid = threadIdx.x, wave = tid >> 6, lane = tid & 63;
  const int r = lane & 15, g = lane >> 4;
  const long m0 = ((long)blockIdx.x * 4 + wave) * (16 * MS);
  const int nb = blockIdx.y;
  const v4i* wsrc = wp + (long)nb * KS * 4 * 64;
  const int total = KS * 256;
  for (int i0 = tid; i0 < total; i0 += 6 * 256) {
    v4i v[6];
#pragma unroll
    for (int k = 0; k < 6; k++) v[k] = wsrc[min(i0 + k * 256, total - 1)];
#pragma unroll
    for (int k = 0; k < 6; k++)
      if (i0 + k * 256 < total) wpanel[i0 + k * 256] = v[k];
  }
  const int8_t* p[MS];
  EpiRegs er[MS];
#pragma unroll
  for (int s = 0; s < MS; s++) {
    const long mc = min(m0 + 16 * s + r, M - 1);
    p[s] = x + mc * K + 16 * g;
    load_epi(er[s], e, ra, mc, N, nb, g);
  }
  v4i aq[PD][MS];
#pragma unroll
  for (int i = 0; i < PD; i++) {
    const int kn = min(i, KS - 1);
#pragma unroll
    for (int s = 0; s < MS; s++) aq[i][s] = ld16(p[s] + 64 * kn);
  }
  v4i acc[MS][4];
#pragma unroll
  for (int s = 0; s < MS; s++)
#pragma unroll
    for (int t = 0; t < 4; t++) acc[s][t] = (v4i){0, 0, 0, 0};
  __syncthreads();
  const v4i* wl = wpanel + lane;
  for (int ks0 = 0; ks0 < KS; ks0 += PD) {
#pragma unroll
    for (int j = 0; j < PD; j++) {
      const int ks = ks0 + j;
      if (ks < KS) {
#pragma unroll
        for (int t = 0; t < 4; t++) {
          const v4i wv = wl[(ks * 4 + t) * 64];
#pragma unroll
          for (int s = 0; s < MS; s++) acc[s][t] = __builtin_amdgcn_mfma_i32_16x16x64_i8(wv, aq[j][s], acc[s][t], 0, 0, 0);
        }
      }
      const int kn = min(ks + PD, KS - 1);
#pragma unroll
      for (int s = 0; s < MS; s++) aq[j][s] = ld16(p[s] + 64 * kn);
    }
  }
#pragma unroll
  for (int s = 0; s < MS; s++) {
    const long m = m0 + 16 * s + r;
    if (m < M) store_tile_e(acc[s], er[s], e, ra, out, m, N, nb, g);
  }
}

template <int NB, int MS, int PD>
__global__ __launch_bounds__(256) void pw_f_kernel(const int8_t* __restrict__ x, const v4i* __restrict__ wp, Epi e, ResArgs ra,
                                                   int8_t* __restrict__ out, long M, int K, int KS, int N, int ) {
  static_assert(PD % 2 == 0, "the activation queue is refilled in pairs of K-steps");
  __shared__ v4i wbuf[2][NB * 4][64];
  const int wave = threadIdx.x >> 6, lane = threadIdx.x & 63;
  const int r = lane & 15, g = lane >> 4;
  const long m0 = ((long)blockIdx.x * 4 + wave) * (16 * MS);
  const int8_t* p[MS];
#pragma unroll
  for (int s = 0; s < MS; s++) p[s] = x + min(m0 + 16 * s + r, M - 1) * K + 16 * g;
  const v4i* w = wp + wave * 64 + lane;
  const long wblk = (long)KS * 4 * 64;
  v4i wst[NB], wnx[NB];
#pragma unroll
  for (int b = 0; b < NB; b++) wst[b] = w[b * wblk];
  const int k1 = min(1, KS - 1);
#pragma unroll
  for (int b = 0; b < NB; b++) wnx[b] = w[b * wblk + (long)k1 * 4 * 64];
  v4i aq[PD][MS];
#pragma unroll
  for (int i = 0; i < PD; i++) {
    const int kn = min(i, KS - 1);
#pragma unroll
    for (int s = 0; s < MS; s++) aq[i][s] = ld16(p[s] + 64 * kn);
  }
  v4i acc[MS][NB][4];
#pragma unroll
  for (int s = 0; s < MS; s++)
#pragma unroll
    for (int b = 0; b < NB; b++)
#pragma unroll
      for (int t = 0; t < 4; t++) acc[s][b][t] = (v4i){0, 0, 0, 0};
#pragma unroll
  for (int b = 0; b < NB; b++) wbuf[0][b * 4 + wave][lane] = wst[b];
#pragma unroll
  for (int b = 0; b < NB; b++) wst[b] = wnx[b];
  __syncthreads();
  for (int ks0 = 0; ks0 < KS; ks0 += PD) {
#pragma unroll
    for (int j = 0; j < PD; j++) {
      const int ks = ks0 + j;
      const int kw = min(ks + 2, KS - 1);
#pragma unroll
      for (int b = 0; b < NB; b++) wnx[b] = w[b * wblk + (long)kw * 4 * 64];
      asm volatile("" ::: "memory");
      if (ks < KS) {
#pragma unroll
        for (int b = 0; b < NB; b++)
#pragma unroll
          for (int t = 0; t < 4; t++) {
            const v4i wv = wbuf[ks & 1][b * 4 + t][lane];
#pragma unroll
            for (int s = 0; s < MS; s++) acc[s][b][t] = __builtin_amdgcn_mfma_i32_16x16x64_i8(wv, aq[j][s], acc[s][b][t], 0, 0, 0);
          }
      }
      if (j & 1) {
        const int kn0 = min(ks - 1 + PD, KS - 1), kn = min(ks + PD, KS - 1);
#pragma unroll
        for (int s = 0; s < MS; s++) { aq[j - 1][s] = ld16(p[s] + 64 * kn0); aq[j][s] = ld16(p[s] + 64 * kn); }
      }
#pragma unroll
      for (int b = 0; b < NB; b++) wbuf[(ks + 1) & 1][b * 4 + wave][lane] = wst[b];
#pragma unroll
      for (int b = 0; b < NB; b++) wst[b] = wnx[b];
      __syncthreads();
    }
  }
#pragma unroll
  for (int b = 0; b < NB; b++)
#pragma unroll
    for (int s = 0; s < MS; s++) {
      const long m = m0 + 16 * s + r;
      EpiRegs er;
      load_epi(er, e, ra, min(m, M - 1), N, b, g);
      if (m < M) store_tile_e(acc[s][b], er, e, ra, out, m, N, b, g);
    }
}

__device__ __forceinline__ unsigned max4_s8(unsigned a, unsigned b) {
  unsigned r = 0;
#pragma unroll
  for (int j = 0; j < 4; j++) {
    int x = (int)(int8_t)(a >> (8 * j)), y = (int)(int8_t)(b >> (8 * j));
    r |= (unsigned)(max(x, y) & 255) << (8 * j);
  }
  return r;
}

constexpr int PWM_MAX = 8;
struct PwProb {
  const int8_t* x;
  const v4i* wp;
  const int* bias;
  const float* mult;
  int8_t* out;
  Rq rq;
  int M, K, KS, N, NB;
  int8_t* pool1;
  int8_t* pool2;
  int H, W, H1, W1, pt1, pl1, H2, W2, pt2, pl2;
};
struct PwMulti {
  int n;
  int start[PWM_MAX + 1];
  PwProb p[PWM_MAX];
};

__device__ __forceinline__ void pwm_pool(const unsigned char* src, int H, int W, int N, int OH, int OW, int pt, int pl, int8_t* gout,
                                         unsigned char* lout, int tid) {
  const int N4 = N >> 2, total = OH * OW * N4;
  const float rcp_n4 = frcp(N4), rcp_ow = frcp(OW);
  for (int i = tid; i < total; i += 256) {
    const int pix = fdiv_small(i, rcp_n4), c4 = i - pix * N4;
    const int oy = fdiv_small(pix, rcp_ow), ox = pix - oy * OW;
    unsigned best = 0x80808080u;
#pragma unroll
    for (int ky = 0; ky < 3; ky++) {
      const int iy = oy * 2 + ky - pt;
#pragma unroll
      for (int kx = 0; kx < 3; kx++) {
        const int ix = ox * 2 + kx - pl;
        if (iy >= 0 && iy < H && ix >= 0 && ix < W) best = max4_s8(best, *(const unsigned*)(src + (iy * W + ix) * N + 4 * c4));
      }
    }
    *(unsigned*)(gout + (long)pix * N + 4 * c4) = best;
    if (lout) *(unsigned*)(lout + pix * N + 4 * c4) = best;
  }
}

__global__ __launch_bounds__(256) void pw_multi_kernel(PwMulti pm) {
  extern __shared__ __attribute__((aligned(16))) unsigned char pwm_smem[];
  const int tid = threadIdx.x, wave = tid >> 6, lane = tid & 63, r = lane & 15, g = lane >> 4;
  int pi = 0;
#pragma unroll
  for (int i = 1; i < PWM_MAX; i++) pi += (i < pm.n && (int)blockIdx.x >= pm.start[i]) ? 1 : 0;
  const PwProb& q = pm.p[pi];
  const int local = blockIdx.x - pm.start[pi];
  const Epi e{q.bias, q.mult, 0, 0, 0, q.rq};
  const ResArgs ra{nullptr, AddQ{0, 0, 0, 0, 0, 0, 0}};
  if (q.pool1 == nullptr) {
    const int nb = local % q.NB;
    const long m0 = ((long)(local / q.NB) * 4 + wave) * 16;
    if (m0 >= q.M) return;
    const long m = min(m0 + r, (long)q.M - 1);
    const int8_t* px = q.x + m * q.K + 16 * g;
    EpiRegs er;
    load_epi(er, e, ra, m, q.N, nb, g);
    v4i acc[4];
#pragma unroll
    for (int t = 0; t < 4; t++) acc[t] = (v4i){0, 0, 0, 0};
    const v4i* w = q.wp + (long)nb * q.KS * 4 * 64 + lane;
#pragma unroll 4
    for (int ks = 0; ks < q.KS; ks++) {
      const v4i av = ld16(px + 64 * ks);
#pragma unroll
      for (int t = 0; t < 4; t++) acc[t] = __builtin_amdgcn_mfma_i32_16x16x64_i8(w[(ks * 4 + t) * 64], av, acc[t], 0, 0, 0);
    }
    if (m0 + r < q.M) store_tile_e(acc, er, e, ra, q.out, m0 + r, q.N, nb, g);
    return;
// ... 796 lines not shown
```

### vbt_amd/csrc/planner.hip

```cpp
#include <algorithm>
#include <cmath>
#include <cstdlib>
#include <functional>
#include <initializer_list>

#include "detector_model.h"
#include "weight_pack.h"

namespace vbt {

static int conv_kb(const vbt_model* m, const OpRec& op) {
  const bool off = getenv("VBT_NO_KBIAS") != nullptr;
  if (off || (op.type != OP_STEM && op.type != OP_PW && op.type != OP_DW)) return 0;
  const TensorRec& tin = m->tensors[op.inputs[0]];
  const TensorRec& tout = m->tensors[op.output];
  const int8_t* w = (const int8_t*)(m->blob.data() + op.w_off);
  const int32_t* bq = (const int32_t*)(m->blob.data() + op.b_off);
  const bool dw = op.type == OP_DW;
  const int N = tout.c, K = dw ? op.k * op.k : op.k * op.k * tin.c;
  for (int co = 0; co < N; co++) {
    long long sa = 0;
    for (int k = 0; k < K; k++) sa += std::abs((int)(dw ? w[(size_t)k * N + co] : w[(size_t)co * K + k]));
    if (255 * sa + std::llabs((long long)bq[co]) >= (1ll << 22) - 1) return 0;
  }
// ... 56 lines not shown
    for (int t = 0; t < kk; t++)
      for (int i = 0; i < 64 && 64 * c + i < Ce; i++) R[ib.o_dw + t * 64 + i] = (unsigned char)wd[(size_t)t * Ce + 64 * c + i];
    for (int nb = 0; nb < NB; nb++)
      for (int k2 = 0; k2 < 2; k2++)
        memcpy(R + ib.o_wp + (size_t)((nb * 2 + k2) * 4) * 512, pp.data() + ((size_t)(nb * (Cp / 32) + 2 * c + k2) * 4) * 64, 4 * 512);
  }
  unsigned char* drec;
  int rc;
  if ((rc = upload(m, rec, &drec))) return rc;
  ib.data = drec;
  *out = ib;
  return VBT_OK;
}

static int make_fused(vbt_model* m, int e_op, int d_op, int p_op, int a_op, Step* out, int sum_op = -1, const NodeSrc* ns = nullptr) {
  const OpRec& dop = m->ops[d_op];
  const OpRec& pop = m->ops[p_op];
  const bool expand = e_op >= 0;
  const int in_t = expand ? m->ops[e_op].inputs[0] : dop.inputs[0];
  const TensorRec& tin = m->tensors[in_t];
  const TensorRec& tdin = m->tensors[dop.inputs[0]];
  const TensorRec& tdout = m->tensors[dop.output];
  const TensorRec& tout = m->tensors[pop.output];
  const int Ce = tdin.c, Cp = (Ce + 63) / 64 * 64, kk = dop.k * dop.k;
  const int8_t* wd = (const int8_t*)(m->blob.data() + dop.w_off);
  const int32_t* bqd = (const int32_t*)(m->blob.data() + dop.b_off);
  const int8_t* wpj = (const int8_t*)(m->blob.data() + pop.w_off);
  int rc;
  Step s;
  s.family = expand ? F_MBCONV : (sum_op >= 0 ? F_NODE : F_SEPCONV);
  s.sum_op = sum_op;
  s.op = a_op >= 0 ? a_op : p_op;
  s.e_op = e_op; s.d_op = d_op; s.p_op = p_op; s.a_op = a_op;
  FusedArgs& a = s.fa;
  memset(&a, 0, sizeof(a));
  a.H = tin.h; a.W = tin.w; a.Cin = tin.c; a.OH = tout.h; a.OW = tout.w; a.Cout = tout.c;
  a.pad_t = dop.pad_t; a.pad_l = dop.pad_l;
  choose_tile(tout.h, tout.w, dop.k, dop.stride, expand, &a.TX, &a.TY);
  a.tiles_x = (tout.w + a.TX - 1) / a.TX;
  a.tiles_y = (tout.h + a.TY - 1) / a.TY;
  a.nchunks = Cp / 64;
  a.zx = tin.zero_point;
  const Step& ps = m->op_steps[p_op];
  s.nbp = ps.NB <= 3 ? ps.NB : 5;
  if (expand) {
    const Step& es = m->op_steps[e_op];
    const OpRec& eop = m->ops[e_op];
    a.we = es.wp; a.be = es.bias; a.me = es.mult; a.KSe = es.KS;
    a.ze = tdin.zero_point; a.loe = eop.act_min; a.hie = eop.act_max;
    a.rqe = make_rq(a.ze, a.loe, a.hie, conv_kb(m, eop));
    a.T0S = ((tin.c + 7) & ~7) + 8;
  } else {
    a.T0S = Cp + 16;
  }
  {
    float* dwf; int* dbias; float* dmult;
    if ((rc = upload(m, dw_weights_f32(wd, Ce, kk, Cp), &dwf)) || (rc = upload(m, fold_bias(bqd, wd, Ce, kk, 128 + tdin.zero_point, W_TAPS, Cp), &dbias)) ||
        (rc = upload(m, pad_floats((const float*)(m->blob.data() + dop.m_off), Ce, Cp), &dmult)))
      return rc;
    a.wd = dwf; a.bd = dbias; a.md = dmult;
    long* dwdm; int* dbm;
    if ((rc = upload(m, pack_dw_diag(wd, Ce, kk, 64), &dwdm)) || (rc = upload(m, fold_bias(bqd, wd, Ce, kk, tdin.zero_point, W_TAPS, Cp), &dbm))) return rc;
    a.wdm = dwdm; a.bdm = dbm;
    if (expand && (dop.k == 3 || dop.k == 5)) {
      const std::vector<v4i> w64 = pack_dw64(wd, Ce, dop.k, Cp / 16);
      v4i* d64; long* d64c;
      if ((rc = upload(m, w64, &d64)) || (rc = upload(m, pack_dw64_compact(w64, dop.k), &d64c))) return rc;
      a.wd64 = d64; a.wd64c = d64c;
      if (fused_tpz_built(dop.k, dop.stride, s.nbp, a.KSe, false)) {
        unsigned* dtz;
        if ((rc = upload(m, pack_expdw2_taps(wd, Ce, 0, Cp / 4, dop.k, dop.stride), &dtz))) return rc;
        a.wtz = dtz;
      }
    }
    a.zd = tdout.zero_point; a.lod = dop.act_min; a.hid = dop.act_max;
    a.rqd = make_rq(a.zd, a.lod, a.hid, conv_kb(m, dop));
  }
  {
    std::vector<v4i> wp;
    pack_weights64(wpj, tout.c, Ce, Cp / 64, s.nbp, wp);
    v4i* dwp;
    if ((rc = upload(m, wp, &dwp))) return rc;
    a.wp = dwp; a.bp = ps.bias; a.mp = ps.mult; a.KSp = Cp / 64;
    a.zo = tout.zero_point; a.lop = pop.act_min; a.hip = pop.act_max;
    a.rqp = make_rq(a.zo, a.lop, a.hip);
  }
  if (a_op >= 0) {
    a.has_res = 1;
    a.resq = m->op_steps[a_op].addq;
  }
  if (sum_op >= 0) {
    fill_node_sources(a, *ns, m, sum_op);
    for (int j = 0; j < ns->n; j++) s.src_tensor[j] = ns->tensor[j];
  }
  s.lds_bytes = fused_tile_lds(a, dop.k, dop.stride, a.TX, a.TY, expand ? FB_EST : 0, 1, s.nbp);
  s.cost = cost_of(m, {e_op, d_op, p_op, a_op, sum_op}, ns);
  if (expand && Ce % 48 == 0 && Ce % 64 != 0) {
    const int8_t* we = (const int8_t*)(m->blob.data() + m->ops[e_op].w_off);
    const int nch3 = Ce / 48;
    const std::vector<int> kmap = kmap48(Ce);
    std::vector<v4i> wp3;
    pack_weights64(wpj, tout.c, Ce, nch3, s.nbp, wp3, &kmap);
    long *d1, *d2;
    v4i* d3;
    if ((rc = upload(m, pack_expand48(we, Ce, tin.c, a.KSe), &d1)) || (rc = upload(m, pack_dw_diag(wd, Ce, kk, 48), &d2)) || (rc = upload(m, wp3, &d3))) return rc;
    a.we3 = d1; a.wdm3 = d2; a.wp3 = d3; a.nch3 = nch3; a.KSp3 = nch3;
  }
  if (expand && tin.h * tin.w <= 400 && tout.h * tout.w <= 400 && (rc = make_image_bundle(m, e_op, d_op, p_op, a.KSe, &s.ib))) return rc;
  *out = s;
  return VBT_OK;
}

static const Alt* tile_alt(const Group& g, int family) {
  for (int i = (int)g.alts.size() - 1; i >= 0; i--)
    if (g.alts[i].steps.size() == 1 && g.alts[i].steps[0].family == family) return &g.alts[i];
  return nullptr;
}
static const Alt* band_alt(const Group& g) {
  for (int i = (int)g.alts.size() - 1; i >= 0; i--)
    if (g.alts[i].steps.size() == 1 && g.alts[i].steps[0].family == F_BAND && g.alts[i].steps[0].members.empty()) return &g.alts[i];
  return nullptr;
}

static bool band_ok(const vbt_model* m, int d_op, int p_op) {
  if (m->flags & VBT_MODEL_NO_BAND) return false;
  if (const char* ns = getenv("VBT_SUBSTREAMS")) if (atoi(ns) > 1) return false;
  const OpRec& d = m->ops[d_op];
  const OpRec& p = m->ops[p_op];
  const TensorRec& ti = m->tensors[d.inputs[0]];
  const TensorRec& to = m->tensors[p.output];
  return d.k == 3 && d.stride == 1 && d.pad_t == 1 && d.pad_l == 1 && ti.c % 8 == 0 && ti.c >= 16 && ti.c <= 128 && to.c <= 128 && to.h == ti.h &&
         to.w == ti.w && ti.w <= 160;
}
static int make_band(vbt_model* m, int d_op, int p_op, int sum_op, const NodeSrc* ns, Step* out) {
  const OpRec& dop = m->ops[d_op];
  const OpRec& pop = m->ops[p_op];
  const TensorRec& tin = m->tensors[dop.inputs[0]];
  const TensorRec& td = m->tensors[dop.output];
  const TensorRec& to = m->tensors[pop.output];
  Step s;
  s.family = F_BAND;
  s.op = p_op;
  s.d_op = d_op;
  s.p_op = p_op;
  s.sum_op = sum_op;
  BandArgs& a = s.bd_args;
  memset(&a, 0, sizeof(a));
  a.H = tin.h; a.W = tin.w; a.Cout = to.c;
  const int C = tin.c;
  a.C = C;
  a.CS = ((C + 15) / 16 | 1) * 16;
  a.NCG = (C + 15) / 16;
  a.KS = (C + 63) / 64;
  static const int band_px_env = getenv("VBT_BAND_PX") ? atoi(getenv("VBT_BAND_PX")) : 0;
  const int band_px = band_px_env > 0 ? band_px_env : (m->max_batch <= 8 ? 64 : 320);
  const int nb = std::max(1, (tin.h * tin.w + band_px - 1) / band_px);
  a.rows = (tin.h + nb - 1) / nb;
  a.nbands = (tin.h + a.rows - 1) / a.rows;
  a.zx4 = (unsigned)(tin.zero_point & 255) * 0x01010101u;
  const int8_t* wd = (const int8_t*)(m->blob.data() + dop.w_off);
  v4i *dpd, *dpp, *dpc = nullptr;
  int* dbd;
  float* dmd;
  int rc;
  if ((rc = upload(m, pack_band_dw(wd, C), &dpd)) || (rc = upload(m, pack_band_pw((const int8_t*)(m->blob.data() + pop.w_off), to.c, C), &dpp)) ||
      (rc = upload(m, fold_bias((const int32_t*)(m->blob.data() + dop.b_off), wd, C, 9, tin.zero_point, W_TAPS, a.NCG * 16), &dbd)) ||
      (rc = upload(m, pad_floats((const float*)(m->blob.data() + dop.m_off), C, a.NCG * 16), &dmd)))
    return rc;
  if (C == 64 && to.c <= 64 && (rc = upload(m, pack_band_pw_chain((const int8_t*)(m->blob.data() + pop.w_off), to.c, C), &dpc))) return rc;
  a.wd = dpd; a.wp = dpp; a.wpc = dpc; a.bd = dbd; a.md = dmd;
  a.bp = m->op_steps[p_op].bias;
  a.mp = m->op_steps[p_op].mult;
  a.rqd = make_rq(td.zero_point, dop.act_min, dop.act_max, conv_kb(m, dop));
  a.rqp = make_rq(to.zero_point, pop.act_min, pop.act_max, conv_kb(m, pop));
  a.x = m->tptr[dop.inputs[0]];
  a.out = m->tptr[pop.output];
  if (sum_op >= 0) {
    fill_node_sources(a, *ns, m, sum_op);
    a.x = nullptr;
    for (int j = 0; j < ns->n; j++) a.src[j] = m->tptr[ns->tensor[j]];
  }
  s.band_tiles = a.nbands;
  s.lds_bytes = band_lds(a);
  std::vector<BandArgs> one{a};
  if ((rc = upload(m, one, &s.d_band))) return rc;
  s.cost = cost_of(m, {d_op, p_op, sum_op}, ns);
  *out = s;
  return VBT_OK;
}
// ... 716 lines not shown
    for (int k : {bk1, bk2}) {
      merged.members.push_back(m->steps[k]);
      merged.cost += m->steps[k].cost;
      drop[k] = 1;
    }
  }
  std::vector<Step> out;
  for (int i = 0; i < ns; i++) {
    if (i == best) out.push_back(merged);
    else if (!drop[i]) out.push_back(m->steps[i]);
  }
  m->steps.swap(out);
}

void finalize_plan(vbt_model* m) {
  m->steps.clear();
  m->materialized.assign(m->tensors.size(), 1);
  for (const Group& g : m->groups) {
    const Alt& a = g.alts[g.chosen];
    for (const Step& s : a.steps) m->steps.push_back(s);
    for (int t : a.hidden) m->materialized[t] = 0;
  }
  merge_side_convs(m);
}

int build_plan(vbt_model* m) {
  const int no = (int)m->ops.size();
  for (int oi = 0; oi < no; oi++) {
    const OpRec& op = m->ops[oi];
    const TensorRec& to = m->tensors[op.output];
    Step s;
    s.op = oi;
    double in_el = 0;
    for (int i = 0; i < op.n_inputs; i++) {
      const TensorRec& ti = m->tensors[op.inputs[i]];
      in_el += (double)ti.h * ti.w * ti.c;
    }
    double out_el = (double)to.h * to.w * to.c;
    s.cost.alg_bytes_per_frame = in_el + out_el;
    if (op.type == OP_STEM || op.type == OP_PW || op.type == OP_DW) {
      const TensorRec& ti = m->tensors[op.inputs[0]];
      const int8_t* w = (const int8_t*)(m->blob.data() + op.w_off);
      const int32_t* bq = (const int32_t*)(m->blob.data() + op.b_off);
      const float* mu = (const float*)(m->blob.data() + op.m_off);
      const int N = to.c;
      const int zx = ti.zero_point;
      if (op.type == OP_DW) {
        s.family = F_DW;
        const int C = N, kk = op.k * op.k;
        if (C % 4 != 0 || !((op.k == 3 || op.k == 5) && (op.stride == 1 || op.stride == 2))) {
          set_error("unsupported depthwise conv: C=%d k=%d s=%d", C, op.k, op.stride);
          return VBT_ERR_ARG;
        }
        int rc;
        if ((rc = upload(m, dw_weights_f32(w, C, kk, C), &s.wf)) || (rc = upload(m, fold_bias(bq, w, C, kk, 128 + zx, W_TAPS), &s.bias)) ||
            (rc = upload(m, pad_floats(mu, C, C), &s.mult)))
          return rc;
        const int Cp = (C + 63) / 64 * 64;
        if ((rc = upload(m, pack_dw_diag(w, C, kk, 64), &s.wdm)) || (rc = upload(m, fold_bias(bq, w, C, kk, zx, W_TAPS, Cp), &s.bdm)) ||
            (rc = upload(m, pad_floats(mu, C, Cp), &s.mdm)))
          return rc;
        s.cost.weight_bytes = (double)kk * C;
        s.cost.macs_per_frame = out_el * kk;
      } else {
        const bool stem = op.type == OP_STEM;
        s.family = stem ? F_STEM : F_PW;
        const int K = stem ? op.k * op.k * ti.c : ti.c;
        if (stem && (op.k != 3 || ti.c != 3 || op.stride != 2)) { set_error("unsupported stem conv"); return VBT_ERR_ARG; }
        if (!stem && (K % 8) != 0) { set_error("pointwise conv needs Cin %% 8 == 0 (got %d)", K); return VBT_ERR_ARG; }
        s.KS = (K + 31) / 32;
        s.NB = (N + 63) / 64;
        const std::vector<int> kmap = stem_kmap();
        std::vector<long> wp;
        pack_weights(w, N, K, s.KS, s.NB, stem ? &kmap : nullptr, wp);
        int rc;
        if ((rc = upload(m, wp, &s.wp)) || (rc = upload(m, fold_bias(bq, w, N, K, zx, W_ROWS, s.NB * 64), &s.bias)) ||
            (rc = upload(m, pad_floats(mu, N, s.NB * 64), &s.mult)))
          return rc;
        if (!stem) {
          s.KS64 = (K + 63) / 64;
          std::vector<v4i> wp64;
          pack_weights64(w, N, K, s.KS64, s.NB, wp64);
          if ((rc = upload(m, wp64, &s.wp64))) return rc;
        }
        s.cost.weight_bytes = (double)N * K;
        s.cost.macs_per_frame = out_el * K;
      }
    } else if (op.type == OP_ADD) {
      s.family = F_ADD;
      if (((long)to.h * to.w * to.c) % 4 != 0 || op.n_inputs != 2) { set_error("unsupported add (binary int8 ADD on a multiple of 4 elements expected)"); return VBT_ERR_ARG; }
      const TensorRec& ta = m->tensors[op.inputs[0]];
      const TensorRec& tb = m->tensors[op.inputs[1]];
      AddParams ap;
      if (!xnn_add_params(ta.scale, tb.scale, to.scale, ta.zero_point, tb.zero_point, &ap)) {
        set_error("op %d: ADD input/output scale ratio outside [2^-10, 2^8) (XNNPACK refuses it too)", oi);
        return VBT_ERR_ARG;
      }
      if (ap.bias != op.add_q[0] || ap.am != op.add_q[1] || ap.bm != op.add_q[2] || ap.shift != op.add_q[3]) {
        set_error("op %d: ADD parameters stored in the container (%d,%d,%d,%d) differ from those derived from the tensor scales (%d,%d,%d,%d)",
                  oi, op.add_q[0], op.add_q[1], op.add_q[2], op.add_q[3], ap.bias, ap.am, ap.bm, ap.shift);
        return VBT_ERR_ARG;
      }
      s.addq = make_addq(ap, to.zero_point, op.act_min, op.act_max);
      auto sole_add_consumer = [&](int t) {
        int n = 0, add = 0;
        for (const OpRec& o2 : m->ops)
          for (int i = 0; i < o2.n_inputs; i++)
            if (o2.inputs[i] == t) { n++; add += o2.type == OP_ADD; }
        return n == 1 && add == 1;
      };
      if (sole_add_consumer(op.output)) s.cost.alg_bytes_per_frame -= out_el;
      for (int i = 0; i < 2; i++) {
        bool from_add = false;
        for (int o2 = 0; o2 < oi; o2++) from_add |= m->ops[o2].type == OP_ADD && m->ops[o2].output == op.inputs[i];
        if (from_add && sole_add_consumer(op.inputs[i])) s.cost.alg_bytes_per_frame -= (double)m->tensors[op.inputs[i]].h * m->tensors[op.inputs[i]].w * m->tensors[op.inputs[i]].c;
      }
    } else if (op.type == OP_MAXPOOL) {
      s.family = F_MAXPOOL;
      if (to.c % 4 != 0 || op.k != 3 || op.stride != 2) { set_error("unsupported maxpool"); return VBT_ERR_ARG; }
    } else if (op.type == OP_RESIZE_NN) {
      s.family = F_RESIZE;
      if (to.c % 4 != 0) { set_error("unsupported resize"); return VBT_ERR_ARG; }
      const TensorRec& ti = m->tensors[op.inputs[0]];
      for (int ax = 0; ax < 2; ax++) {
        const int in = ax ? ti.w : ti.h, out = ax ? to.w : to.h;
        const float scale = (float)in / (float)out;
        for (int d = 0; d < out; d++)
          if (std::min((int)floorf((float)d * scale), in - 1) != (d * in) / out) {
            set_error("op %d: nearest-neighbour resize %d -> %d is not mapped", oi, in, out);
            return VBT_ERR_ARG;
          }
      }
    } else if (op.type == OP_POSTPROCESS) {
      s.family = F_POST;
      if (op.n_inputs != 10 || m->hdr.max_detections != VBT_MAX_DETECTIONS || m->hdr.num_anchors > 65535) {
        set_error("unsupported postprocess configuration");
        return VBT_ERR_ARG;
      }
      s.cost.alg_bytes_per_frame = in_el + m->hdr.max_detections * 24.0;
      s.cost.weight_bytes = (double)m->hdr.num_anchors * 16;
    } else {
      set_error("unknown op type %d", op.type);
      return VBT_ERR_ARG;
    }
    m->op_steps.push_back(s);
  }
  return fuse_plan(m);
}

}
```

### vbt_amd/csrc/weight_pack.h

```cpp
#pragma once
#include <algorithm>
#include <cstdint>
#include <vector>
#ifdef __HIP__
#include "dev_common.h"
using vbt::v4i;
#endif

inline void pack_weights(const int8_t* w, int N, int K, int KS, int NB, const std::vector<int>* kmap, std::vector<long>& out) {
  out.assign((size_t)NB * KS * 4 * 64, 0);
  int8_t* o = (int8_t*)out.data();
  for (int nb = 0; nb < NB; nb++)
    for (int ks = 0; ks < KS; ks++)
      for (int t = 0; t < 4; t++)
        for (int lane = 0; lane < 64; lane++) {
          int i = lane & 15, g = lane >> 4;
          int co = 64 * nb + 16 * (i >> 2) + 4 * t + (i & 3);
          for (int j = 0; j < 8; j++) {
            int kp = 32 * ks + 8 * g + j;
            int k = kmap ? (kp < (int)kmap->size() ? (*kmap)[kp] : -1) : (kp < K ? kp : -1);
            int8_t v = (co < N && k >= 0) ? w[(size_t)co * K + k] : 0;
            o[((((size_t)(nb * KS + ks) * 4 + t) * 64 + lane) * 8) + j] = v;
          }
        }
}

inline void pack_weights64(const int8_t* w, int N, int K, int KS, int NB, std::vector<v4i>& out, const std::vector<int>* kmap = nullptr) {
  out.assign((size_t)NB * KS * 4 * 64, (v4i){0, 0, 0, 0});
  int8_t* o = (int8_t*)out.data();
  for (int nb = 0; nb < NB; nb++)
    for (int ks = 0; ks < KS; ks++)
      for (int t = 0; t < 4; t++)
        for (int lane = 0; lane < 64; lane++) {
          const int i = lane & 15, g = lane >> 4, co = 64 * nb + 16 * (i >> 2) + 4 * t + (i & 3);
          for (int j = 0; j < 16; j++) {
            const int kp = 64 * ks + 16 * g + j;
            const int k = kmap ? (kp < (int)kmap->size() ? (*kmap)[kp] : -1) : (kp < K ? kp : -1);
            o[((((size_t)(nb * KS + ks) * 4 + t) * 64 + lane) * 16) + j] = (co < N && k >= 0) ? w[(size_t)co * K + k] : 0;
          }
        }
}

enum WLayout { W_ROWS, W_TAPS };
inline std::vector<int> fold_bias(const int32_t* bq, const int8_t* w, int n, int K, int zp, WLayout layout, int padded = 0) {
  std::vector<int> out(std::max(n, padded), 0);
  for (int c = 0; c < n; c++) {
    long sw = 0;
    for (int k = 0; k < K; k++) sw += layout == W_ROWS ? w[(size_t)c * K + k] : w[(size_t)k * n + c];
    out[c] = (int)((long)bq[c] - (long)zp * sw);
  }
  return out;
}
template <typename T>
inline std::vector<float> pad_floats(const T* v, int n, int padded) {
  std::vector<float> out(std::max(n, padded), 0.0f);
  for (int c = 0; c < n; c++) out[c] = (float)v[c];
  return out;
}
inline std::vector<float> dw_weights_f32(const int8_t* w, int C, int kk, int Cp) {
  std::vector<float> out((size_t)kk * Cp, 0.0f);
  for (int t = 0; t < kk; t++)
    for (int c = 0; c < C; c++) out[(size_t)t * Cp + c] = (float)w[(size_t)t * C + c];
  return out;
}

inline std::vector<long> pack_dw_diag(const int8_t* w, int C, int kk, int group_channels) {
  const int NCG = group_channels / 16, nch = (C + group_channels - 1) / group_channels, KT = (kk + 1) / 2;
  std::vector<long> out((size_t)nch * NCG * KT * 64, 0);
  int8_t* o = (int8_t*)out.data();
  for (int ch = 0; ch < nch; ch++)
    for (int cg = 0; cg < NCG; cg++)
      for (int mi = 0; mi < KT; mi++)
        for (int lane = 0; lane < 64; lane++) {
          const int i = lane & 15, g = lane >> 4, c = group_channels * ch + 16 * cg + i, tap = 2 * mi + (g >> 1);
          for (int j = 0; j < 8; j++)
            o[((((size_t)(ch * NCG + cg) * KT + mi) * 64 + lane) * 8) + j] = (tap < kk && 8 * (g & 1) + j == i && c < C) ? w[(size_t)tap * C + c] : 0;
        }
  return out;
}

inline std::vector<v4i> pack_dw64(const int8_t* w, int C, int k, int nq) {
  const int K64 = k == 3 ? 3 : 7;
  std::vector<v4i> out((size_t)nq * K64 * 64, (v4i){0, 0, 0, 0});
  int8_t* o = (int8_t*)out.data();
  for (int q = 0; q < nq; q++)
    for (int mi = 0; mi < K64; mi++)
      for (int lane = 0; lane < 64; lane++) {
        const int i = lane & 15, g = lane >> 4, c = 16 * q + i;
        int tap = -1;
        if (k == 3) tap = g < 3 ? mi * 3 + g : -1;
        else if (mi < 5) tap = mi * 5 + g;
        else if (mi == 5) tap = g * 5 + 4;
        else tap = g == 0 ? 24 : -1;
        if (tap >= 0 && c < C) o[(((size_t)q * K64 + mi) * 64 + lane) * 16 + i] = w[(size_t)tap * C + c];
      }
  return out;
}
inline std::vector<long> pack_dw64_compact(const std::vector<v4i>& w64, int k) {
  const int K64 = k == 3 ? 3 : 7, nq = (int)(w64.size() / ((size_t)K64 * 64));
  std::vector<long> out((size_t)nq * 64, 0);
  const int8_t* o = (const int8_t*)w64.data();
  int8_t* oc = (int8_t*)out.data();
  for (int q = 0; q < nq; q++)
    for (int mi = 0; mi < K64; mi++)
      for (int lane = 0; lane < 64; lane++)
        oc[((size_t)q * 64 + lane) * 8 + mi] = o[(((size_t)q * K64 + mi) * 64 + lane) * 16 + (lane & 15)];
  return out;
}

inline std::vector<long> pack_expand48(const int8_t* w, int Ce, int K, int KS) {
  const int nch3 = Ce / 48;
  std::vector<long> out((size_t)nch3 * KS * 3 * 64, 0);
  int8_t* o = (int8_t*)out.data();
  for (int c = 0; c < nch3; c++)
    for (int ks = 0; ks < KS; ks++)
      for (int t = 0; t < 3; t++)
        for (int lane = 0; lane < 64; lane++) {
          const int i = lane & 15, kg = lane >> 4, co = 48 * c + 12 * (i >> 2) + 4 * t + (i & 3);
          for (int j = 0; j < 8; j++) {
            const int k = 32 * ks + 8 * kg + j;
            o[((((size_t)(c * KS + ks) * 3 + t) * 64 + lane) * 8) + j] = k < K ? w[(size_t)co * K + k] : 0;
          }
        }
// ... 150 lines not shown
```

### vbt_amd/interpreter.py

```python
import ctypes
import os

import numpy as np

from . import _lib

MAXDET = 25


class Interpreter:
    def __init__(self, model_path, num_threads=4, device=0, max_batch=1, fuse=True, flags=None):
        self.model_path = str(model_path)
        self.num_threads = num_threads
        self.device = device
        self.max_batch = int(max_batch)
        self._h = ctypes.c_void_p()
        if flags is None:
            flags = int(os.environ.get('VBT_FUSION_FLAGS', '0')) if fuse else 1
        from .tflite_import import as_container_path
        path, temporary = as_container_path(self.model_path)
        try:
            _lib.check(_lib.lib().vbt_model_create_ex(path.encode(), device, self.max_batch, flags, ctypes.byref(self._h)))
        finally:
            if temporary:
                os.unlink(path)
        shp = (ctypes.c_int * 4)()
        _lib.check(_lib.lib().vbt_model_input_shape(self._h, shp))
        self._shape = np.array([1, shp[1], shp[2], shp[3]], dtype=np.int32)

    @classmethod
    def _borrowed(cls, handle, model_path, device, max_batch, owner):
        self = cls.__new__(cls)
        self.model_path, self.num_threads, self.device, self.max_batch = str(model_path), 4, device, int(max_batch)
        self._h, self._owner = ctypes.c_void_p(handle), owner
        shp = (ctypes.c_int * 4)()
        _lib.check(_lib.lib().vbt_model_input_shape(self._h, shp))
        self._shape = np.array([1, shp[1], shp[2], shp[3]], dtype=np.int32)
        return self

    def __del__(self):
        h = getattr(self, "_h", None)
        if h and getattr(self, "_owner", None) is None and _lib is not None and _lib._lib is not None:
            _lib._lib.vbt_model_destroy(h)
            self._h = None

    @property
    def handle(self):
        return self._h

    def allocate_tensors(self):
        return None

    def get_input_details(self):
        return [{"name": "images", "index": 0, "shape": self._shape.copy(), "dtype": np.uint8}]

    def get_signature_runner(self, signature_key=None):
        def run(images):
            images = np.asarray(images)
            if images.dtype != np.uint8 or images.ndim != 4 or tuple(images.shape[1:]) != tuple(self._shape[1:]):
                raise ValueError(f"images must be uint8 [B,{self._shape[1]},{self._shape[2]},3], got {images.dtype} {images.shape}")
            boxes, scores, classes, counts = self.detect(images)
            if images.shape[0] == 1:
                return {"output_0": counts.astype(np.float32), "output_1": scores, "output_2": classes, "output_3": boxes}
            return {"output_0": counts.astype(np.float32), "output_1": scores, "output_2": classes, "output_3": boxes}
        return run

    def detect(self, frames):
        frames = np.ascontiguousarray(frames, dtype=np.uint8)
        B = frames.shape[0]
        boxes = np.empty((B, MAXDET, 4), np.float32)
        scores = np.empty((B, MAXDET), np.float32)
        classes = np.empty((B, MAXDET), np.float32)
        counts = np.empty((B,), np.int32)
        _lib.check(_lib.lib().vbt_detect(self._h, frames.ctypes.data, B, 0, None, boxes.ctypes.data, scores.ctypes.data,
                                         classes.ctypes.data, counts.ctypes.data, 0))
        return boxes, scores, classes, counts

    def num_tensors(self):
        return _lib.lib().vbt_model_num_tensors(self._h)

    def materialized(self, tid):
        return bool(_lib.lib().vbt_model_tensor_materialized(self._h, tid))

    def num_launches(self):
        return _lib.lib().vbt_model_num_launches(self._h)

    def plan_space(self):
        n = ctypes.c_int()
        rc = _lib.lib().vbt_model_plan_space(self._h, None, 0, ctypes.byref(n))
        if rc not in (0, -4):
            _lib.check(rc)
        buf = (_lib.PlanStepSpace * max(n.value, 1))()
        _lib.check(_lib.lib().vbt_model_plan_space(self._h, buf, n.value, ctypes.byref(n)))
        return [{"group": e.group, "alt": e.alt, "step": e.step, "chosen": bool(e.chosen), "variant": e.variant, "first_op": e.first_op,
                 "last_op": e.last_op, "family": e.family.decode(), "variants": list(e.variants[:e.n_variants])} for e in buf[:n.value]]

    def read_tensor(self, tid, B):
        shp = (ctypes.c_int * 3)()
        _lib.check(_lib.lib().vbt_model_tensor_shape(self._h, tid, shp))
        out = np.empty((B, shp[0], shp[1], shp[2]), np.int8)
        _lib.check(_lib.lib().vbt_model_read_tensor(self._h, tid, B, out.ctypes.data))
        return out
```

Measured before the change: 125,100.

## Pack partial last output block tile-major to skip dead MFMA tiles in projections

Adds a tile-major packing for the last 64-channel output block of pointwise and MBConv projection convolutions whose channel count is not a multiple of 64. Only the live 16-channel tiles of that block are computed, with new template instantiations for the fused MBConv kernel and two new autotuner variants for the all-blocks pointwise kernel. The aim is to stop issuing MFMAs, weight loads and LDS traffic for zero-padded output channels. The cost is extra kernel instantiations, an extra packed copy of the weights, and a separate epilogue path for the tail tiles.

Result: faster. 128,700, median of 6 (+3.0%).

```diff
diff --git a/include/vbt_hip_diag.h b/include/vbt_hip_diag.h
--- a/include/vbt_hip_diag.h
+++ b/include/vbt_hip_diag.h
@@ -38,6 +38,7 @@
   int variants[48];
 } vbt_plan_step_space;
 int vbt_model_plan_space(const vbt_model* m, vbt_plan_step_space* out, int cap, int* n);
+int vbt_model_step_proj_tail(const vbt_model* m, int group, int alt, int step);
 
 int vbt_streams_share_queue(void* a, void* b, int us, int* shared);
 
diff --git a/vbt_amd/_lib.py b/vbt_amd/_lib.py
--- a/vbt_amd/_lib.py
+++ b/vbt_amd/_lib.py
@@ -122,6 +122,7 @@
     "vbt_streams_share_queue": (c_int, [c_void_p, c_void_p, c_int, c_void_p]),
     "vbt_model_read_tensor": (c_int, [c_void_p, c_int, c_int, c_void_p]),
     "vbt_model_plan_space": (c_int, [c_void_p, c_void_p, c_int, ctypes.POINTER(c_int)]),
+    "vbt_model_step_proj_tail": (c_int, [c_void_p, c_int, c_int, c_int]),
     "vbt_resize_frames": (c_int, [c_void_p, c_int, c_int, c_int, c_int, c_void_p, c_int, c_int, c_int, c_int, c_int, c_void_p]),
     "vbt_resize_frames_yuv": (c_int, [c_void_p, c_int, c_int, c_int, c_int, c_int, c_void_p, c_int, c_int, c_int, c_int, c_void_p]),
     "vbt_model_kernel_stats": (c_int, [c_void_p, c_int, ctypes.POINTER(KernelStat), c_int, ctypes.POINTER(c_int)]),
diff --git a/vbt_amd/csrc/detector.hip b/vbt_amd/csrc/detector.hip
--- a/vbt_amd/csrc/detector.hip
+++ b/vbt_amd/csrc/detector.hip
@@ -1,5 +1,6 @@
 #include <algorithm>
 #include <cmath>
+#include <string>
 
 #include "detector_model.h"
 #include "op_kernels.h"
@@ -25,15 +26,18 @@
     return L;
   }
   static const int pw_force = getenv("VBT_PW_VARIANT") ? atoi(getenv("VBT_PW_VARIANT")) : -100;
-  const bool f_fits = s.NB >= 2 && s.NB <= PW_F_MAX_NB;
-  if (pw_force != -100 && (f_fits || (pw_force != 7 && pw_force != 8))) variant = pw_force;
-  if (variant == 7 || variant == 8) {
+  const bool f_fits = s.NB >= 2 && s.NB <= PW_F_MAX_NB, ft_fits = f_fits && s.wp64t && pw_f_tail_built(s.NB, s.ntl);
+  if (pw_force != -100 && (pw_force == 9 || pw_force == 10 ? ft_fits : (f_fits || (pw_force != 7 && pw_force != 8)))) variant = pw_force;
+  if (variant >= 7 && variant <= 10) {
+    const bool tail = variant >= 9;
     L.form = PW_F;
-    L.ms = variant - 6;
-    L.lds = s.NB * 8192;
+    L.ms = tail ? variant - 8 : variant - 6;
+    L.ntl = tail ? s.ntl : 0;
+    L.lds = tail ? (4 * (s.NB - 1) + s.ntl) * 2048 : s.NB * 8192;
     L.grid = dim3((unsigned)((M + 64 * L.ms - 1) / (64 * L.ms)), 1);
     if (s.NB < 2) L.refuse(VBT_ERR_ARG, "pw_conv: one output block - nothing for the all-blocks form to share");
     else if (s.NB > PW_F_MAX_NB) L.refuse(VBT_ERR_ARG, "pw_conv: %d output blocks exceed the %d whose accumulators the all-blocks form holds", s.NB, PW_F_MAX_NB);
+    else if (tail && !ft_fits) L.refuse(VBT_ERR_ARG, "pw_conv: no tile-major last block for %d output blocks with %d tail tiles", s.NB, s.ntl);
   } else if (variant >= 3 && variant <= 6) {
     L.form = variant <= 4 ? PW_D : PW_E;
     L.ms = 2 - (variant & 1);
@@ -75,7 +79,14 @@
       break;
     case PW_F:
 #define PW_F_NB(NBF) (L.ms == 2 ? PW((pw_f_kernel<NBF, 2, 4>), 0) : PW((pw_f_kernel<NBF, 1, 4>), 0))
-      if (s.NB == 2) PW_F_NB(2); else if (s.NB == 3) PW_F_NB(3); else if (s.NB == 4) PW_F_NB(4); else if (s.NB == 5) PW_F_NB(5); else PW_F_NB(6);
+#define PW_F_TAIL(NBF, NTL) (L.ms == 2 ? pw_f_kernel<NBF, 2, 4, NTL><<<L.grid, 256, 0, st>>>(x, s.wp64t, e, ra, out, M, K, s.KS64, N, s.NB) \
+                                     : pw_f_kernel<NBF, 1, 4, NTL><<<L.grid, 256, 0, st>>>(x, s.wp64t, e, ra, out, M, K, s.KS64, N, s.NB))
+      if (L.ntl) {
+        if (s.NB == 2 && L.ntl == 1) PW_F_TAIL(2, 1); else if (s.NB == 2 && L.ntl == 2) PW_F_TAIL(2, 2); else if (s.NB == 2 && L.ntl == 3) PW_F_TAIL(2, 3);
+        else if (s.NB == 2) PW_F_TAIL(2, 4); else if (s.NB == 4) PW_F_TAIL(4, 1); else PW_F_TAIL(6, 2);
+      }
+      else if (s.NB == 2) PW_F_NB(2); else if (s.NB == 3) PW_F_NB(3); else if (s.NB == 4) PW_F_NB(4); else if (s.NB == 5) PW_F_NB(5); else PW_F_NB(6);
+#undef PW_F_TAIL
 #undef PW_F_NB
       break;
     case PW_B:
@@ -140,6 +151,11 @@
   return VBT_OK;
 }
 
+static bool proj_tail_on(int block) {
+  static const std::string knob = getenv("VBT_PROJ_TAIL") ? std::string(",") + getenv("VBT_PROJ_TAIL") + "," : std::string();
+  if (knob.empty()) return true;
+  return knob.find(",b" + std::to_string(block) + ",") != std::string::npos;
+}
 FusedPlan resolve_fused(const vbt_model* m, const Step& s, int variant, int B) {
   const FusedArgs& a = s.fa;
   const OpRec& dop = m->ops[s.d_op];
@@ -183,6 +199,7 @@
   p.tiles_y = (a.OH + p.TY - 1) / p.TY;
   p.L = FusedLaunch{k, stride, s.nbp, ex, mdw, nt3, ppw2, dw64, fused_tile_lds(a, k, stride, p.TX, p.TY, est, ppw2 ? 2 : 1, s.nbp, e_bytes),
                     (unsigned)((long)B * p.tiles_x * p.tiles_y), tpz_ok};
+  if (s.ntl && proj_tail_on(s.block) && (nt3 ? a.wpt3 : a.wpt) && fused_tail_built(p.L, a.KSe, s.ntl)) p.L.ntl = s.ntl;
   if (ppw2 && (a.OW < 16 || a.OH < 8 || !a.wd64)) p.refuse(VBT_ERR_ARG, "fused_mbconv: the 128-pixel variant needs maps of at least 16 x 8");
   else if (ppw2 && p.L.lds_bytes > 64 * 1024) p.refuse(VBT_ERR_ARG, "fused_mbconv: 128-pixel tile needs %d bytes of LDS", p.L.lds_bytes);
   else if (tpz && !tpz_ok) p.refuse(VBT_ERR_ARG, "fused_mbconv: variant %d: the Toeplitz depthwise does not apply to this step", var);
diff --git a/vbt_amd/csrc/detector_model.h b/vbt_amd/csrc/detector_model.h
--- a/vbt_amd/csrc/detector_model.h
+++ b/vbt_amd/csrc/detector_model.h
@@ -29,6 +29,8 @@
   long* wp = nullptr;
   v4i* wp64 = nullptr;
   int KS64 = 0;
+  v4i* wp64t = nullptr;
+  int ntl = 0;
   int res_op = -1;
   long* wdm = nullptr;
   int* bdm = nullptr;
@@ -44,6 +46,7 @@
   int src_tensor[3] = {-1, -1, -1};
   FusedArgs fa;
   int nbp = 0, lds_bytes = 0;
+  int block = 0;
   int variant = -1;
   double tuned_ms = 0;
   std::vector<Step> members;
@@ -144,7 +147,8 @@
 };
 enum PwForm { PW_A, PW_B, PW_C, PW_D, PW_E, PW_F };
 constexpr int PW_F_MAX_NB = 6;
-struct PwLaunch : Verdict { PwForm form = PW_B; int ms = 1, nbt = 1, nb_per_y = 0, lds = 0; dim3 grid; };
+static inline bool pw_f_tail_built(int NB, int ntl) { return (NB == 2 && ntl >= 1 && ntl <= 4) || (NB == 4 && ntl == 1) || (NB == 6 && ntl == 2); }
+struct PwLaunch : Verdict { PwForm form = PW_B; int ms = 1, nbt = 1, nb_per_y = 0, lds = 0, ntl = 0; dim3 grid; };
 enum DwForm { DW_ROW, DW_COL, DW_TILE };
 struct DwLaunch : Verdict {
   DwForm form = DW_COL; bool mdw = false; int TX = 0, TY = 0, tiles_x = 0, tiles_y = 0, lds = 0, rows = 0, nseg = 0; long total = 0; dim3 grid;
diff --git a/vbt_amd/csrc/detector_plan.hip b/vbt_amd/csrc/detector_plan.hip
--- a/vbt_amd/csrc/detector_plan.hip
+++ b/vbt_amd/csrc/detector_plan.hip
@@ -123,7 +123,7 @@
   } else if (st.family == F_PW && st.KS64 <= 4) {
     cand = {0, 1};
   } else if (st.family == F_PW) {
-    cand = {-1, 2, 3, 4, 5, 6, 7, 8};
+    cand = {-1, 2, 3, 4, 5, 6, 7, 8, 9, 10};
   } else if (is_fused_tile(st.family)) {
     cand = {0, 1, 3, 5};
     if (st.family == F_MBCONV && st.fa.nch3 > 0 && st.nbp <= 2 && st.fa.KSe >= 1 && st.fa.KSe <= 4) { cand.push_back(9); cand.push_back(11); }
@@ -303,6 +303,15 @@
         std::copy(ps.variants.begin(), ps.variants.end(), o.variants);
       }
   return VBT_OK;
+}
+
+int vbt_model_step_proj_tail(const vbt_model* m, int group, int alt, int step) {
+  if (!m || group < 0 || group >= (int)m->groups.size() || alt < 0 || alt >= (int)m->groups[group].alts.size() || step < 0 ||
+      step >= (int)m->groups[group].alts[alt].steps.size()) { set_error("vbt_model_step_proj_tail: no such step"); return VBT_ERR_ARG; }
+  const Step& st = m->groups[group].alts[alt].steps[step];
+  if (st.family == F_MBCONV) { const FusedPlan p = resolve_fused(m, st, st.variant, m->max_batch); return p.rc ? 0 : p.L.ntl; }
+  if (st.family == F_PW && st.members.empty()) { const PwLaunch L = resolve_pw(m, st, st.variant, m->max_batch); return L.rc ? 0 : L.ntl; }
+  return 0;
 }
 
 int vbt_model_create_ex(const char* path, int device, int max_batch, int flags, vbt_model** out) {
diff --git a/vbt_amd/csrc/fused_block.h b/vbt_amd/csrc/fused_block.h
--- a/vbt_amd/csrc/fused_block.h
+++ b/vbt_amd/csrc/fused_block.h
@@ -30,6 +30,8 @@
   const long* wd64c;
   const unsigned* wtz;
   const v4i* wp;
+  const v4i* wpt;
+  const v4i* wpt3;
   const int* bp;
   const float* mp;
   int KSp, zo, lop, hip;
@@ -63,9 +65,11 @@
 constexpr int FB_EST = 80;
 constexpr int FB_DST = 80;
 
-template <int KK, int S, int NBP, bool EXPAND, bool MDW, int KSE = 0, int NT = 4, int PPW = 1, bool DW64 = false, bool TPZ = false>
+template <int KK, int S, int NBP, bool EXPAND, bool MDW, int KSE = 0, int NT = 4, int PPW = 1, bool DW64 = false, bool TPZ = false, int NTL = 0>
 __device__ __forceinline__ void fused_block_body(const FusedArgs& a, int tile, unsigned char* fb_smem) {
   static_assert(PPW == 1 || MDW, "128-pixel tiles exist for the matrix-pipe depthwise only");
+  static_assert(NTL >= 0 && NTL <= 4 && (NTL == 0 || EXPAND), "a tile-major last block (MBConv only) holds one to four tiles");
+  constexpr int NBW = NTL ? NBP - 1 : NBP;
   static_assert(!DW64 || (EXPAND && MDW && (KK == 3 || KK == 5)), "DW64: fused expand blocks, 3x3 / 5x5");
   static_assert(!TPZ || (DW64 && (S == 1 || S == 2) && (NT == 3 || NT == 4) && NBP <= 2 && (KSE == 1 || KSE == 2)), "TPZ: a form of DW64");
   constexpr TpzGeom TG = TPZ ? tpz_geom(KK, S, PPW, NT) : TpzGeom{};
@@ -492,14 +496,24 @@
         bv[pp] = *(const v4i*)(D + (TPZ ? tpz_d_slot(TG, PPW, FB_DST, slot) : slot * FB_DST) + 16 * g);
       }
 #pragma unroll
-      for (int nb = 0; nb < NBP; nb++) {
+      for (int nb = 0; nb < NBW; nb++) {
         const v4i* w = stage_p ? (const v4i*)WPS + (nb * 4) * 64 + lane
+                               : NTL ? (NT == 3 ? a.wpt3 + ((long)(nb * a.KSp3 + c) * 4) * 64 : a.wpt + ((long)(nb * a.KSp + c) * 4) * 64) + lane
                                : (NT == 3 ? a.wp3 + ((long)(nb * a.KSp3 + c) * 4) * 64 : a.wp + ((long)(nb * a.KSp + c) * 4) * 64) + lane;
 #pragma unroll
         for (int t = 0; t < 4; t++) {
           const v4i wv = w[t * 64];
 #pragma unroll
           for (int pp = 0; pp < PPW; pp++) acc[pp][nb][t] = __builtin_amdgcn_mfma_i32_16x16x64_i8(wv, bv[pp], acc[pp][nb][t], 0, 0, 0);
+        }
+      }
+      if constexpr (NTL > 0) {
+        const v4i* w = (NT == 3 ? a.wpt3 + ((long)NBW * a.KSp3 * 4 + (long)c * NTL) * 64 : a.wpt + ((long)NBW * a.KSp * 4 + (long)c * NTL) * 64) + lane;
+#pragma unroll
+        for (int t = 0; t < NTL; t++) {
+          const v4i wv = w[t * 64];
+#pragma unroll
+          for (int pp = 0; pp < PPW; pp++) acc[pp][NBW][t] = __builtin_amdgcn_mfma_i32_16x16x64_i8(wv, bv[pp], acc[pp][NBW][t], 0, 0, 0);
         }
       }
     }
@@ -514,8 +528,19 @@
   if (py < a.TY && px < a.TX && oy < a.OH && ox < a.OW) {
     const unsigned char* skip = T0 + ((py + a.pad_t) * HWx + (px + a.pad_l)) * a.T0S;
     int8_t* orow = a.out + ((b * a.OH + oy) * (long)a.OW + ox) * a.Cout;
-#pragma unroll
-    for (int nb = 0; nb < NBP; nb++) {
+    if constexpr (NTL > 0) {
+#pragma unroll
+      for (int t = 0; t < NTL; t++) {
+        const int c = NBW * 64 + 16 * t + 4 * g;
+        const int4 bb = *(const int4*)(a.bp + c);
+        const float4 mu = *(const float4*)(a.mp + c);
+        unsigned dq = rq_pack_i(acc[pp][NBW][t], bb, mu, a.rqp);
+        if (a.has_res) dq = addq4(dq, *(const unsigned*)(skip + min(c, a.Cin - 4)), a.resq);
+        if (c < a.Cout) *(unsigned*)(orow + c) = dq;
+      }
+    }
+#pragma unroll
+    for (int nb = 0; nb < NBW; nb++) {
       const int c0 = nb * 64 + 16 * g;
       if (c0 >= a.Cout) continue;
       unsigned d[4];
@@ -560,10 +585,10 @@
 #ifndef FB_MINW
 #define FB_MINW 1
 #endif
-template <int KK, int S, int NBP, bool EXPAND, bool MDW, int KSE = 0, int NT = 4, int PPW = 1, bool DW64 = false, bool TPZ = false>
+template <int KK, int S, int NBP, bool EXPAND, bool MDW, int KSE = 0, int NT = 4, int PPW = 1, bool DW64 = false, bool TPZ = false, int NTL = 0>
 __global__ __launch_bounds__(256, FB_MINW) void fused_block_kernel(FusedArgs a) {
   extern __shared__ __attribute__((aligned(16))) unsigned char fb_smem_dyn[];
-  fused_block_body<KK, S, NBP, EXPAND, MDW, KSE, NT, PPW, DW64, TPZ>(a, blockIdx.x, fb_smem_dyn);
+  fused_block_body<KK, S, NBP, EXPAND, MDW, KSE, NT, PPW, DW64, TPZ, NTL>(a, blockIdx.x, fb_smem_dyn);
 }
 
 struct MultiTiles {
diff --git a/vbt_amd/csrc/k_fused_mbconv.hip b/vbt_amd/csrc/k_fused_mbconv.hip
--- a/vbt_amd/csrc/k_fused_mbconv.hip
+++ b/vbt_amd/csrc/k_fused_mbconv.hip
@@ -47,7 +47,10 @@
 
 int launch_fused_mbconv_tpz(const FusedArgs& a, const FusedLaunch& L, hipStream_t st);
 
+int launch_fused_mbconv_tail(const FusedArgs& a, const FusedLaunch& L, hipStream_t st);
+
 int launch_fused_mbconv(const FusedArgs& a, const FusedLaunch& L, hipStream_t st) {
+  if (L.ntl) return launch_fused_mbconv_tail(a, L, st);
   if (L.tpz) return launch_fused_mbconv_tpz(a, L, st);
   const dim3 grid(L.grid);
   if (L.ppw2) {
diff --git a/vbt_amd/csrc/k_fused_mbconv_tail.hip b/vbt_amd/csrc/k_fused_mbconv_tail.hip
--- /dev/null
+++ b/vbt_amd/csrc/k_fused_mbconv_tail.hip
@@ -0,0 +1,41 @@
+#include "launchers.h"
+
+namespace vbt {
+
+#define FB_TAIL1(KK, S, KSE, NTL)                                                             \
+  do {                                                                                                                            \
+    if (L.nt3) fused_block_kernel<KK, S, 1, true, true, KSE, 3, 1, true, true, NTL><<<grid, 256, L.lds_bytes, st>>>(a);           \
+    else fused_block_kernel<KK, S, 1, true, true, KSE, 4, 1, true, true, NTL><<<grid, 256, L.lds_bytes, st>>>(a);                 \
+    return VBT_OK;                                                                                                                \
+  } while (0)
+#define FB_TAIL2(KK, S, KSE, NTL)                                                            \
+  do {                                                                                                                            \
+    if (L.nt3) fused_block_kernel<KK, S, 1, true, true, KSE, 3, 2, true, true, NTL><<<grid, 256, L.lds_bytes, st>>>(a);           \
+    else fused_block_kernel<KK, S, 1, true, true, KSE, 4, 2, true, true, NTL><<<grid, 256, L.lds_bytes, st>>>(a);                 \
+    return VBT_OK;                                                                                                                \
+  } while (0)
+#define FB_TAIL(KK, S, KSE, NTL) do { if (L.ppw2) FB_TAIL2(KK, S, KSE, NTL); else FB_TAIL1(KK, S, KSE, NTL); } while (0)
+
+int launch_fused_mbconv_tail(const FusedArgs& a, const FusedLaunch& L, hipStream_t st) {
+  const dim3 grid(L.grid);
+  const int k = L.k, s = L.stride, kse = a.KSe;
+  if (fused_tail_built(L, kse, L.ntl) && (L.nt3 ? a.wpt3 : a.wpt)) {
+    if (L.tpz && a.wtz) {
+      if (k == 3 && s == 2 && kse == 1) FB_TAIL(3, 2, 1, 2);
+      if (k == 3 && s == 1 && kse == 1) FB_TAIL(3, 1, 1, 2);
+      if (k == 5 && s == 2 && kse == 1) FB_TAIL1(5, 2, 1, 3);
+      if (k == 5 && s == 1 && kse == 2) FB_TAIL(5, 1, 2, 3);
+    } else if (!L.tpz && L.dw64) {
+      if (k == 3) fused_block_kernel<3, 2, 1, true, true, 1, 3, 1, true, false, 2><<<grid, 256, L.lds_bytes, st>>>(a);
+      else fused_block_kernel<5, 2, 1, true, true, 1, 3, 1, true, false, 3><<<grid, 256, L.lds_bytes, st>>>(a);
+      return VBT_OK;
+    } else if (!L.tpz) {
+      fused_block_kernel<3, 2, 2, true, true, 2, 4, 1, false, false, 1><<<grid, 256, L.lds_bytes, st>>>(a);
+      return VBT_OK;
+    }
+  }
+  set_error("fused_mbconv: no instantiation with %d live tiles in the last projection block for k=%d s=%d nbp=%d KSe=%d", L.ntl, k, s, L.nbp, kse);
+  return VBT_ERR_ARG;
+}
+
+}
diff --git a/vbt_amd/csrc/launchers.h b/vbt_amd/csrc/launchers.h
--- a/vbt_amd/csrc/launchers.h
+++ b/vbt_amd/csrc/launchers.h
@@ -19,10 +19,16 @@
   int lds_bytes;
   unsigned grid;
   bool tpz = false;
+  int ntl = 0;
 };
 static inline bool fused_tpz_built(int k, int stride, int nbp, int kse, bool ppw2) {
   return (k == 3 && stride == 2 && nbp == 1 && kse == 1) || (k == 3 && stride == 1 && nbp == 1 && kse == 1) ||
          (k == 5 && stride == 2 && nbp == 1 && kse == 1 && !ppw2) || (k == 5 && stride == 1 && nbp == 1 && kse == 2);
+}
+static inline bool fused_tail_built(const FusedLaunch& L, int kse, int ntl) {
+  if (L.tpz) return fused_tpz_built(L.k, L.stride, L.nbp, kse, L.ppw2) && ntl == (L.k == 3 ? 2 : 3);
+  if (L.dw64) return L.nt3 && !L.ppw2 && L.stride == 2 && L.nbp == 1 && kse == 1 && ntl == (L.k == 3 ? 2 : 3);
+  return L.expand && L.mdw && !L.nt3 && !L.ppw2 && !L.dw64 && L.k == 3 && L.stride == 2 && L.nbp == 2 && kse == 2 && ntl == 1;
 }
 int launch_fused_block(const FusedArgs& a, const FusedLaunch& L, hipStream_t st);
 int launch_fused_multi(const FusedArgs* d_args, const MultiTiles& mt, int k, int stride, int nbp, bool mdw, int lds_bytes, unsigned grid,
diff --git a/vbt_amd/csrc/op_kernels.h b/vbt_amd/csrc/op_kernels.h
--- a/vbt_amd/csrc/op_kernels.h
+++ b/vbt_amd/csrc/op_kernels.h
@@ -82,6 +82,21 @@
 #pragma unroll
       for (int j = 0; j < 4; j++)
         if (c0 + 4 * t + j < N) o[4 * t + j] = (int8_t)(d[t] >> (8 * j));
+  }
+}
+template <int NTL>
+__device__ __forceinline__ void store_tail_tiles(const v4i acc[4], const Epi& e, const ResArgs& ra, int8_t* __restrict__ out, long m, int N,
+                                                 int nb, int g) {
+#pragma unroll
+  for (int t = 0; t < NTL; t++) {
+    const int c = nb * 64 + 16 * t + 4 * g;
+    const int4 b = *(const int4*)(e.bias + c);
+    const float4 mu = *(const float4*)(e.mult + c);
+    if (c < N) {
+      unsigned d = rq_pack_i(acc[t], b, mu, e.rq);
+      if (ra.res) d = addq4(d, *(const unsigned*)(ra.res + m * N + c), ra.q);
+      *(unsigned*)(out + m * N + c) = d;
+    }
   }
 }
 __device__ __forceinline__ v4i ld16(const int8_t* p) {
@@ -366,12 +381,16 @@
   }
 }
 
-template <int NB, int MS, int PD>
+template <int NB, int MS, int PD, int NTL = 0>
 __global__ __launch_bounds__(256) void pw_f_kernel(const int8_t* __restrict__ x, const v4i* __restrict__ wp, Epi e, ResArgs ra,
                                                    int8_t* __restrict__ out, long M, int K, int KS, int N, int ) {
   static_assert(PD % 2 == 0, "the activation queue is refilled in pairs of K-steps");
-  __shared__ v4i wbuf[2][NB * 4][64];
-  const int wave = threadIdx.x >> 6, lane = threadIdx.x & 63;
+  static_assert(NTL >= 0 && NTL <= 4 && (NTL == 0 || NB >= 2), "a tile-major last block holds one to four tiles");
+  constexpr int NBW = NTL ? NB - 1 : NB;
+  constexpr int NTT = 4 * NBW + NTL;
+  __shared__ v4i wbuf[2][NTT][64];
+  const int wave = NTL ? __builtin_amdgcn_readfirstlane(threadIdx.x >> 6) : threadIdx.x >> 6, lane = threadIdx.x & 63;
+  const bool tail_w = wave < NTL;
   const int r = lane & 15, g = lane >> 4;
   const long m0 = ((long)blockIdx.x * 4 + wave) * (16 * MS);
   const int8_t* p[MS];
@@ -379,12 +398,17 @@
   for (int s = 0; s < MS; s++) p[s] = x + min(m0 + 16 * s + r, M - 1) * K + 16 * g;
   const v4i* w = wp + wave * 64 + lane;
   const long wblk = (long)KS * 4 * 64;
+  const v4i* wt = wp + NBW * wblk + wave * 64 + lane;
   v4i wst[NB], wnx[NB];
 #pragma unroll
-  for (int b = 0; b < NB; b++) wst[b] = w[b * wblk];
+  for (int b = 0; b < NBW; b++) wst[b] = w[b * wblk];
   const int k1 = min(1, KS - 1);
 #pragma unroll
-  for (int b = 0; b < NB; b++) wnx[b] = w[b * wblk + (long)k1 * 4 * 64];
+  for (int b = 0; b < NBW; b++) wnx[b] = w[b * wblk + (long)k1 * 4 * 64];
+  if constexpr (NTL > 0) {
+    wst[NBW] = wnx[NBW] = (v4i){0, 0, 0, 0};
+    if (tail_w) { wst[NBW] = wt[0]; wnx[NBW] = wt[(long)k1 * NTL * 64]; }
+  }
   v4i aq[PD][MS];
 #pragma unroll
   for (int i = 0; i < PD; i++) {
@@ -400,7 +424,8 @@
 #pragma unroll
       for (int t = 0; t < 4; t++) acc[s][b][t] = (v4i){0, 0, 0, 0};
 #pragma unroll
-  for (int b = 0; b < NB; b++) wbuf[0][b * 4 + wave][lane] = wst[b];
+  for (int b = 0; b < NBW; b++) wbuf[0][b * 4 + wave][lane] = wst[b];
+  if constexpr (NTL > 0) { if (tail_w) wbuf[0][4 * NBW + wave][lane] = wst[NBW]; }
 #pragma unroll
   for (int b = 0; b < NB; b++) wst[b] = wnx[b];
   __syncthreads();
@@ -410,13 +435,14 @@
       const int ks = ks0 + j;
       const int kw = min(ks + 2, KS - 1);
 #pragma unroll
-      for (int b = 0; b < NB; b++) wnx[b] = w[b * wblk + (long)kw * 4 * 64];
+      for (int b = 0; b < NBW; b++) wnx[b] = w[b * wblk + (long)kw * 4 * 64];
+      if constexpr (NTL > 0) { if (tail_w) wnx[NBW] = wt[(long)kw * NTL * 64]; }
       asm volatile("" ::: "memory");
       if (ks < KS) {
 #pragma unroll
         for (int b = 0; b < NB; b++)
 #pragma unroll
-          for (int t = 0; t < 4; t++) {
+          for (int t = 0; t < (b < NBW ? 4 : NTL); t++) {
             const v4i wv = wbuf[ks & 1][b * 4 + t][lane];
 #pragma unroll
             for (int s = 0; s < MS; s++) acc[s][b][t] = __builtin_amdgcn_mfma_i32_16x16x64_i8(wv, aq[j][s], acc[s][b][t], 0, 0, 0);
@@ -428,14 +454,15 @@
         for (int s = 0; s < MS; s++) { aq[j - 1][s] = ld16(p[s] + 64 * kn0); aq[j][s] = ld16(p[s] + 64 * kn); }
       }
 #pragma unroll
-      for (int b = 0; b < NB; b++) wbuf[(ks + 1) & 1][b * 4 + wave][lane] = wst[b];
+      for (int b = 0; b < NBW; b++) wbuf[(ks + 1) & 1][b * 4 + wave][lane] = wst[b];
+      if constexpr (NTL > 0) { if (tail_w) wbuf[(ks + 1) & 1][4 * NBW + wave][lane] = wst[NBW]; }
 #pragma unroll
       for (int b = 0; b < NB; b++) wst[b] = wnx[b];
       __syncthreads();
     }
   }
 #pragma unroll
-  for (int b = 0; b < NB; b++)
+  for (int b = 0; b < NBW; b++)
 #pragma unroll
     for (int s = 0; s < MS; s++) {
       const long m = m0 + 16 * s + r;
@@ -443,6 +470,13 @@
       load_epi(er, e, ra, min(m, M - 1), N, b, g);
       if (m < M) store_tile_e(acc[s][b], er, e, ra, out, m, N, b, g);
     }
+  if constexpr (NTL > 0) {
+#pragma unroll
+    for (int s = 0; s < MS; s++) {
+      const long m = m0 + 16 * s + r;
+      if (m < M) store_tail_tiles<NTL>(acc[s][NBW], e, ra, out, m, N, NBW, g);
+    }
+  }
 }
 
 __device__ __forceinline__ unsigned max4_s8(unsigned a, unsigned b) {
diff --git a/vbt_amd/csrc/planner.hip b/vbt_amd/csrc/planner.hip
--- a/vbt_amd/csrc/planner.hip
+++ b/vbt_amd/csrc/planner.hip
@@ -162,6 +162,13 @@
     v4i* dwp;
     if ((rc = upload(m, wp, &dwp))) return rc;
     a.wp = dwp; a.bp = ps.bias; a.mp = ps.mult; a.KSp = Cp / 64;
+    if (expand && tout.c % 64 != 0 && tout.c % 4 == 0 && s.nbp == (tout.c + 63) / 64) {
+      pack_weights64_tail(wpj, tout.c, Ce, Cp / 64, s.nbp, wp);
+      if ((rc = upload(m, wp, &dwp))) return rc;
+      a.wpt = dwp;
+      s.ntl = proj_tail_tiles(tout.c);
+      for (int i = 0; i < d_op; i++) s.block += m->ops[i].type == OP_DW;
+    }
     a.zo = tout.zero_point; a.lop = pop.act_min; a.hip = pop.act_max;
     a.rqp = make_rq(a.zo, a.lop, a.hip);
   }
@@ -185,6 +192,11 @@
     v4i* d3;
     if ((rc = upload(m, pack_expand48(we, Ce, tin.c, a.KSe), &d1)) || (rc = upload(m, pack_dw_diag(wd, Ce, kk, 48), &d2)) || (rc = upload(m, wp3, &d3))) return rc;
     a.we3 = d1; a.wdm3 = d2; a.wp3 = d3; a.nch3 = nch3; a.KSp3 = nch3;
+    if (s.ntl) {
+      pack_weights64_tail(wpj, tout.c, Ce, nch3, s.nbp, wp3, &kmap);
+      if ((rc = upload(m, wp3, &d3))) return rc;
+      a.wpt3 = d3;
+    }
   }
   if (expand && tin.h * tin.w <= 400 && tout.h * tout.w <= 400 && (rc = make_image_bundle(m, e_op, d_op, p_op, a.KSe, &s.ib))) return rc;
   *out = s;
@@ -1067,6 +1079,11 @@
           std::vector<v4i> wp64;
           pack_weights64(w, N, K, s.KS64, s.NB, wp64);
           if ((rc = upload(m, wp64, &s.wp64))) return rc;
+          if (s.KS64 > 4 && N % 64 != 0 && N % 4 == 0 && pw_f_tail_built(s.NB, proj_tail_tiles(N))) {
+            pack_weights64_tail(w, N, K, s.KS64, s.NB, wp64);
+            if ((rc = upload(m, wp64, &s.wp64t))) return rc;
+            s.ntl = proj_tail_tiles(N);
+          }
         }
         s.cost.weight_bytes = (double)N * K;
         s.cost.macs_per_frame = out_el * K;
diff --git a/vbt_amd/csrc/weight_pack.h b/vbt_amd/csrc/weight_pack.h
--- a/vbt_amd/csrc/weight_pack.h
+++ b/vbt_amd/csrc/weight_pack.h
@@ -39,6 +39,27 @@
             o[((((size_t)(nb * KS + ks) * 4 + t) * 64 + lane) * 16) + j] = (co < N && k >= 0) ? w[(size_t)co * K + k] : 0;
           }
         }
+}
+
+inline int proj_tail_tiles(int N) { return ((N % 64) + 15) / 16; }
+inline void pack_weights64_tail(const int8_t* w, int N, int K, int KS, int NB, std::vector<v4i>& out, const std::vector<int>* kmap = nullptr) {
+  if (N % 64 == 0 || NB != (N + 63) / 64) { pack_weights64(w, N, K, KS, NB, out, kmap); return; }
+  const int NTL = proj_tail_tiles(N), nbl = NB - 1;
+  std::vector<v4i> full;
+  pack_weights64(w, 64 * nbl, K, KS, nbl, full, kmap);
+  out.assign((size_t)nbl * KS * 4 * 64 + (size_t)KS * NTL * 64, (v4i){0, 0, 0, 0});
+  std::copy(full.begin(), full.end(), out.begin());
+  int8_t* o = (int8_t*)(out.data() + (size_t)nbl * KS * 4 * 64);
+  for (int ks = 0; ks < KS; ks++)
+    for (int t = 0; t < NTL; t++)
+      for (int lane = 0; lane < 64; lane++) {
+        const int i = lane & 15, g = lane >> 4, co = 64 * nbl + 16 * t + i;
+        for (int j = 0; j < 16; j++) {
+          const int kp = 64 * ks + 16 * g + j;
+          const int k = kmap ? (kp < (int)kmap->size() ? (*kmap)[kp] : -1) : (kp < K ? kp : -1);
+          o[(((size_t)(ks * NTL + t) * 64 + lane) * 16) + j] = (co < N && k >= 0) ? w[(size_t)co * K + k] : 0;
+        }
+      }
 }
 
 enum WLayout { W_ROWS, W_TAPS };
diff --git a/vbt_amd/interpreter.py b/vbt_amd/interpreter.py
--- a/vbt_amd/interpreter.py
+++ b/vbt_amd/interpreter.py
@@ -95,6 +95,12 @@
         return [{"group": e.group, "alt": e.alt, "step": e.step, "chosen": bool(e.chosen), "variant": e.variant, "first_op": e.first_op,
                  "last_op": e.last_op, "family": e.family.decode(), "variants": list(e.variants[:e.n_variants])} for e in buf[:n.value]]
 
+    def proj_tail(self, group, alt, step):
+        n = _lib.lib().vbt_model_step_proj_tail(self._h, group, alt, step)
+        if n < 0:
+            _lib.check(n)
+        return n
+
     def read_tensor(self, tid, B):
         shp = (ctypes.c_int * 3)()
         _lib.check(_lib.lib().vbt_model_tensor_shape(self._h, tid, shp))
```
